# ekzhang/rpt

Hardware: AMD Instinct MI355X
Metric: Msamples/s (higher is better)
Workload: dtype f64

## Files before the change

rpt_amd/csrc/api_render.cpp:

```cpp
#include "api_internal.h"

namespace rptapi {

int event_pair_begin(rptgpu_scene* h, int kind, bool on) {
  h->stats.kernel_launches[kind]++;
  if (!on || h->ev_used + 2 > MAX_EVENT_PAIRS * 2) return -1;
  while ((int)h->ev_pool.size() < h->ev_used + 2) {
    hipEvent_t e;
    HIP_TRY(hipEventCreate(&e));
    h->ev_pool.push_back(e);
  }
  const int e0 = h->ev_used;
  h->ev_used += 2;
  HIP_TRY(hipEventRecord(h->ev_pool[e0], h->stream));
  return e0;
}
void event_pair_end(rptgpu_scene* h, int kind, int e0) {
  if (e0 < 0) return;
  HIP_TRY(hipEventRecord(h->ev_pool[e0 + 1], h->stream));
  h->pending.push_back({kind, e0, e0 + 1});
}

struct Bracket {
  rptgpu_scene* h;
  int kind, e0;
  Bracket(rptgpu_scene* h_, int kind_, bool on) : h(h_), kind(kind_), e0(event_pair_begin(h_, kind_, on)) {}
  void done() { event_pair_end(h, kind, e0); }
};

struct QueryMarks {
  rptgpu_scene* h;
  bool on;
  int e0[RPT_K_COUNT];
  QueryMarks(rptgpu_scene* h_, bool on_) : h(h_), on(on_) {
    for (int& e : e0) e = -1;
  }
};
void query_mark(void* ctx, int kind, int end) {
  QueryMarks* q = (QueryMarks*)ctx;
  if (kind < 0 || kind >= RPT_K_COUNT) return;
  if (!end) {
    q->e0[kind] = event_pair_begin(q->h, kind, q->on);
  } else {
    event_pair_end(q->h, kind, q->e0[kind]);
    q->e0[kind] = -1;
  }
}

void drain_events(rptgpu_scene* h) {
  for (auto& p : h->pending) {
    float ms = 0;
    HIP_TRY(hipEventElapsedTime(&ms, h->ev_pool[p.e0], h->ev_pool[p.e1]));
    h->stats.kernel_ms[p.kind] += ms;
  }
  h->pending.clear();
  h->ev_used = 0;
}

std::vector<uint32_t> pixel_list(uint32_t width, uint32_t height, uint32_t tw, uint32_t th, uint32_t pi, uint32_t pc) {
  std::vector<uint32_t> pix;
  uint32_t tiles_x = (width + tw - 1) / tw;
  pix.reserve((size_t)width * height / pc + 1);
  for (uint32_t by = 0; by < height; by += 8)
    for (uint32_t bx = 0; bx < width; bx += 8)
      for (uint32_t y = by; y < std::min(by + 8, height); y++)
        for (uint32_t x = bx; x < std::min(bx + 8, width); x++) {
          uint32_t tile = (y / th) * tiles_x + (x / tw);
          if (pc <= 1 || tile % pc == pi) pix.push_back(y * width + x);
        }
  return pix;
}
void ensure_partition(rptgpu_scene* h, const RptRenderParams& p) {
  uint32_t tw = p.tile_width ? p.tile_width : 32, th = p.tile_height ? p.tile_height : 8;
  uint32_t pc = p.part_count ? p.part_count : 1, pi = p.part_count ? p.part_index : 0;
  uint32_t key[6] = {p.width, p.height, tw, th, pi, pc};
  if (std::memcmp(key, h->part_key, sizeof key) == 0 && h->pixels.p) return;
  std::vector<uint32_t> pix = pixel_list(p.width, p.height, tw, th, pi, pc);
  h->pixels.upload(pix, h->stream);
  HIP_TRY(hipStreamSynchronize(h->stream));
  h->npix = (uint32_t)pix.size();
  std::memcpy(h->part_key, key, sizeof key);
}

void ensure_generic(rptgpu_scene* h, bool all) {
  const uint32_t blocks_few = 64, blocks_all = (uint32_t)std::max(64, std::min(1024, h->num_cus * 4));
  const uint32_t want = (all ? blocks_all : blocks_few) * 256u;
  if (h->gen_threads < want) {
    const uint64_t levels = std::max(1u, h->gen_levels), frames = std::max(1u, h->gen_frames);
    h->gen_defer.release(); h->gen_frame.release();
    h->gen_defer.alloc(levels * 8u * want);
    h->gen_frame.alloc(frames * 12u * want);
    h->gen_overflow.alloc(1);
    HIP_TRY(hipMemsetAsync(h->gen_overflow.p, 0, sizeof(uint32_t), h->stream));
    h->gen_threads = want;
  }
  h->spill.gen = GenericStack{h->gen_defer.p, h->gen_frame.p, h->gen_threads, std::max(1u, h->gen_levels), std::max(1u, h->gen_frames)};
  h->spill.gen_overflow = h->gen_overflow.p;
  h->spill.gen_blocks_few = blocks_few;
  h->spill.gen_blocks_all = h->gen_threads / 256u >= blocks_all ? blocks_all : blocks_few;
}

int drain_call(rptgpu_scene* h, bool read_overflow) {
  hipStream_t st = h->stream;
  uint32_t gen_overflow = 0;
  if (read_overflow) HIP_TRY(hipMemcpyAsync(&gen_overflow, h->gen_overflow.p, sizeof gen_overflow, hipMemcpyDeviceToHost, st));
  HIP_TRY(hipStreamSynchronize(st));
  drain_events(h);
  if (gen_overflow) {
    (void)hipMemsetAsync(h->gen_overflow.p, 0, sizeof(uint32_t), st);
    return fail(h, RPTGPU_E_TREE_TOO_DEEP, "rpt_tree_generic: the traversal outgrew the stack sized for this scene (internal error)");
  }
  return RPTGPU_OK;
}

void ensure_sort_bufs(rptgpu_scene* h, uint64_t cap) {
  h->sort_kin.alloc(cap); h->sort_kout.alloc(cap); h->sort_vin.alloc(cap);
  size_t bytes = rpt_strict::TABLE.sort_temp_bytes((uint32_t)cap);
  h->sort_tmp.alloc(bytes);
  h->sort_bufs = SortBufs{h->sort_kin.p, h->sort_kout.p, h->sort_vin.p, h->sort_tmp.p, bytes};
}

uint32_t zeros_common(const std::vector<rptdev::Light>& lights) {
  for (const rptdev::Light& l : lights)
    if (l.kind == RPT_LIGHT_DIRECTIONAL && (l.vec[0] == 0.0 || l.vec[1] == 0.0 || l.vec[2] == 0.0)) return 1;
  return 0;
}

void ensure_workspace(rptgpu_scene* h, uint64_t cap, uint64_t rec_cols) {
  if (cap <= h->ws_cap && rec_cols <= h->ws_rec_cols && h->ray.p) return;
  cap = std::max(cap, h->ws_cap);
  rec_cols = std::max(rec_cols, h->ws_rec_cols);
  int nl = std::max(1, h->dscene.num_lights);
  h->ray.alloc(6 * cap);
  h->hit.alloc(4 * cap);
  h->hit_obj.alloc(cap);
  h->draw.alloc(cap); h->pid.alloc(cap); h->col.alloc(cap);
  if (h->path_reorder) {
    h->next_rows.alloc(8 * cap);
  } else {
    h->ray_next.alloc(6 * cap);
    h->draw_next.alloc(cap); h->pid_next.alloc(cap); h->col_next.alloc(cap);
  }
  h->last_col.alloc(cap);
  h->rec.release();
  h->rec.alloc((uint64_t)rptdev::REC_FIELDS * rec_cols);
  h->rec_parent.alloc(rec_cols);
  h->shadow.release();
  h->shadow.alloc((uint64_t)nl * rptdev::SHADOW_FIELDS * cap);
  h->counters.alloc(2 * (2 + (size_t)nl));
  h->shadow_q.release();
  h->shadow_q.alloc((uint64_t)nl * cap);
  h->srt.release();
  h->srt.alloc((uint64_t)nl * cap);
  if (h->has_deep) {
    h->tq.alloc(3 * cap);
    h->tq_ctr.alloc(16);
    {
      const uint64_t threads = (uint64_t)std::max(1, h->num_cus * 4) / 4 * RPT_TT_WAVES * 256;
      const uint64_t levels = (uint64_t)(std::max<uint32_t>((uint32_t)rptdev::KD_MAX_STACK, h->max_tree_depth + 1u) - RPT_TT_LEVELS_MIN);
      h->spill_node.alloc(levels * threads); h->spill_ts.alloc(levels * threads); h->spill_bmax.alloc(levels * threads);
      h->tree_rays.alloc(8 * cap);
      h->spill = StackSpill{h->spill_node.p, h->spill_ts.p, h->spill_bmax.p, (uint32_t)threads, zeros_common(h->host_lights),
                            h->tree_rays.p};
    }
    ensure_generic(h, h->gen_all);
    if (h->sort_rays) ensure_sort_bufs(h, cap);
  }
  if (h->path_reorder) {
    h->path_order.alloc(cap);
    ensure_sort_bufs(h, cap);
  }
  h->ws_cap = cap;
  h->ws_rec_cols = rec_cols;
}

void print_prof(const KernelTable* kt, const char* what) {
  static const char* const NAMES[29] = {
      "tree_trace refill", "tree_trace node steps", "tree_trace box tests", "tree_trace pop", "tree_trace write-out",
      "tree_trace exact tests", "in-kernel node step", "in-kernel box batch", "in-kernel child test",
      "in-kernel triangle batch", "in-kernel object", "paths fetch", "paths raygen", "paths closest_hit",
      "paths illuminate", "paths visible", "paths nee_bsdf", "paths sample_f", "paths bsdf", "paths record",
      "paths fold+store", "flat candidate walk", "fold iteration", "rejection round", "paths fused query",
      "paths draws", "paths shade block", "pre-trace pass", "pre-trace pass, cubes skipped"};
  unsigned long long t[4][29];
  if (!kt->read_prof(t)) return;
  unsigned long long tot = 0;
  for (int i = 0; i < 29; i++) tot += t[0][i];
  std::fprintf(stderr, "prof[%s] %-28s %8s %10s %14s %10s\n", what, "phase", "time %", "lanes/64", "iterations", "lanes/64");
  for (int i = 0; i < 29; i++) {
    if (!t[0][i] && !t[2][i]) continue;
    char a[32] = "-", b[32] = "-", c[32] = "-", d[32] = "-";
    if (t[0][i]) {
      std::snprintf(a, sizeof a, "%.2f", tot ? 100.0 * (double)t[0][i] / (double)tot : 0.0);
      std::snprintf(b, sizeof b, "%.1f", (double)t[1][i] / (double)t[0][i]);
    }
    if (t[2][i]) {
      std::snprintf(c, sizeof c, "%llu", t[2][i]);
      std::snprintf(d, sizeof d, "%.1f", (double)t[3][i] / (double)t[2][i]);
    }
    std::fprintf(stderr, "prof[%s] %-28s %8s %10s %14s %10s\n", what, NAMES[i], a, b, c, d);
  }
}

void release_workspace(rptgpu_scene* h) {
  h->ray.release(); h->ray_next.release(); h->hit.release(); h->hit_obj.release(); h->draw.release(); h->draw_next.release();
  h->pid.release(); h->pid_next.release(); h->col.release(); h->col_next.release(); h->rec.release();
  h->rec_parent.release(); h->last_col.release();
  h->shadow.release(); h->tq.release(); h->srt.release(); h->shadow_q.release();
  h->sort_kin.release(); h->sort_kout.release(); h->sort_vin.release(); h->sort_tmp.release(); h->tree_rays.release();
  h->path_order.release(); h->next_rows.release();
  h->gen_defer.release(); h->gen_frame.release(); h->gen_threads = 0;
  h->ws_cap = 0; h->ws_rec_cols = 0;
}

rptplan::PassPlan size_pass(rptgpu_scene* h, const rptplan::PassInput& in, uint32_t npix, bool generic_all) {
  rptplan::PassPlan pp = rptplan::plan_pass(in);
  for (;;) {
    const uint64_t np = rptplan::pass_slots(npix, pp);
    try {
      ensure_workspace(h, np, rptplan::pass_rec_cols(np, in.ratio));
      if (generic_all) ensure_generic(h, true);
      return pp;
    } catch (const HipError& e) {
      if (e.e != hipErrorOutOfMemory || pp.s_chunk == 1) throw;
      (void)hipGetLastError();
      release_workspace(h);
      h->ws_fail_paths = rptplan::fail_paths_after_oom(h->ws_fail_paths, np);
      pp = rptplan::shrink_after_oom(pp);
    }
  }
}

void reset_tree_counters(rptgpu_scene* h) {
  HIP_TRY(hipMemsetAsync(h->tq_ctr.p, 0, 16 * sizeof(uint32_t), h->stream));
  h->qtune.ctr_set = 0;
}
static void tree_query(rptgpu_scene* h, const KernelTable* kt, const rptdev::PathState& ps, const uint32_t* queue, uint32_t n,
                       int light, double* srt, const uint32_t* d_n, const QueryHook* hook) {
  kt->query(h->stream, h->dscene, ps, queue, n, light, srt, d_n, h->obj_deep.data(), h->obj_tris.data(), h->dscene.num_objects,
            h->tq.p, h->tq_ctr.p, (uint32_t)std::max(1, h->num_cus * 4), h->sort_rays ? &h->sort_bufs : nullptr, hook, &h->spill,
            &h->qtune);
}
void query_closest(rptgpu_scene* h, const KernelTable* kt, const rptdev::PathState& ps, uint32_t n, const QueryHook* hook) {
  tree_query(h, kt, ps, nullptr, n, -1, nullptr, nullptr, hook);
}
void query_visibility(rptgpu_scene* h, const KernelTable* kt, const rptdev::PathState& ps, int l, uint32_t n,
                      const uint32_t* d_n, const QueryHook* hook) {
  tree_query(h, kt, ps, h->shadow_q.p + (uint64_t)l * ps.cap, n, l, h->srt.p, d_n, hook);
}

rptdev::Camera make_camera(const RptCamera& c) {
  rptdev::Camera d{};
  std::memcpy(d.eye, c.eye, sizeof d.eye);
  std::memcpy(d.direction, c.direction, sizeof d.direction);
  std::memcpy(d.up, c.up, sizeof d.up);
  d.d = 1.0 / std::tan(c.fov / 2.0);
  const double* a = c.direction;
  const double* b = c.up;
  double cr[3] = {a[1] * b[2] - a[2] * b[1], a[2] * b[0] - a[0] * b[2], a[0] * b[1] - a[1] * b[0]};
  double len = std::sqrt((cr[0] * cr[0] + cr[1] * cr[1]) + cr[2] * cr[2]);
  for (int k = 0; k < 3; k++) d.right[k] = cr[k] / len;
  d.aperture = c.aperture;
  d.focal_distance = c.focal_distance;
  return d;
}

const char* bad_params(const RptRenderParams* p) {
  if (!p->width || !p->height || !p->iterations) return "width, height and iterations must be non-zero";
  if (p->max_bounces > 254) return "max_bounces > 254";
  if ((uint64_t)p->width * p->height >= (1ull << 31)) return "frame too large";
  if (p->part_count && p->part_index >= p->part_count) return "part_index >= part_count";
  if (p->precision_mode != RPT_PRECISION_F64_STRICT) return BAD_MODE;
  return nullptr;
}

int64_t free_memory() {
  size_t free_b = 0, total_b = 0;
  return hipMemGetInfo(&free_b, &total_b) == hipSuccess ? (int64_t)free_b : -1;
}

rptdev::PathState path_state(rptgpu_scene* h) {
  rptdev::PathState ps{};
  ps.ray = h->ray.p; ps.hit = h->hit.p; ps.hit_obj = h->hit_obj.p; ps.draw = h->draw.p;
  ps.pid = h->pid.p; ps.col = h->col.p;
  ps.ray_next = h->ray_next.p; ps.draw_next = h->draw_next.p; ps.pid_next = h->pid_next.p; ps.col_next = h->col_next.p;
  ps.rec = h->rec.p; ps.rec_parent = h->rec_parent.p; ps.last_col = h->last_col.p;
  ps.shadow = h->shadow.p; ps.cap = h->ws_cap; ps.rec_cap = h->ws_rec_cols;
  if (h->path_reorder) {
    ps.sort_keys = h->sort_kin.p; ps.sort_vals = h->sort_vin.p; ps.next_rows = h->next_rows.p;
    std::memcpy(ps.key_bounds, h->scene_bounds, sizeof ps.key_bounds);
  }
  return ps;
}

void render_persistent(rptgpu_scene* h, const KernelTable* kt, const RptRenderParams& p, rptdev::Frame fr,
                       const rptdev::Camera& cam, void* out, bool out_f32, bool packed, bool prof) {
  hipStream_t st = h->stream;
  const uint32_t npix = fr.npix;
  const bool print_launch = std::getenv("RPTGPU_PRINT_LAUNCH") != nullptr;
  const uint64_t lbuf_held = h->lbuf.n * sizeof(double);
  const int64_t free_b = lbuf_held < h->lbuf_max_bytes ? free_memory() : -1;
  const bool flat = h->all_flat && !h->dscene.force_general;
  FlatLayout lay = flat ? h->flat_layout : FlatLayout{};
  const uint32_t flat_lds = lay.off_end;
  if (RPT_PRETRACE_CULL && lay.pretrace_cull) {
    for (size_t i = 0; i < h->obj_geom.size() && i < 64 && lay.cull_n < (uint32_t)RPT_CULL_MAX; i++) {
      uint32_t r[4];
      if (((lay.cull_always >> i) & 1ull) ||
          !rpthost::pinhole_screen_rect(rpthost::world_box(h->obj_geom[i], h->top_insts[i]), cam, fr.width, fr.height, r))
        continue;
      lay.cull_obj[lay.cull_n] = (uint32_t)i;
      const bool off = r[0] > r[1] || r[2] > r[3];
      lay.cull_lo[lay.cull_n] = off ? 0xffffffffu : (r[0] | (r[2] << 16));
      lay.cull_ext[lay.cull_n] = off ? 0u : ((r[1] - r[0]) | ((r[3] - r[2]) << 16));
      lay.cull_n++;
    }
  }
  const rptplan::PersistentPlan pl = rptplan::plan_persistent(
      npix, p.iterations, p.max_bounces, h->num_cus, kt->paths_max_blocks_per_cu(flat ? &lay : nullptr, flat_lds, false),
      h->lbuf_max_bytes, lbuf_held, free_b, h->paths_chunk, h->all_flat, h->dscene.force_general, h->flat_layout.obj_filter);
  bool park = flat && h->opt.env_park != 0 && h->dscene.env_kind != RPT_ENV_COLOR;
  if (park && kt->paths_max_blocks_per_cu(&lay, flat_lds, true) < pl.per_cu) park = false;
  h->prec.alloc((uint64_t)rpt_fold_ring_slots(p.max_bounces) * rptdev::REC_FIELDS * ((uint64_t)pl.nblocks * 64));
  h->lbuf.alloc(std::max<uint64_t>(1, (uint64_t)pl.spp_l * 3 * npix));
  if (print_launch)
    std::fprintf(stderr, "rpt_paths<%s>: %d blocks/CU x %d CUs -> %u blocks, %u samples per work item, %u launch(es) of %u spp, "
                 "dynamic LDS %u B per wave (the flat scene's tables)%s%s%s%s\n",
                 flat ? (lay.obj_filter ? "KdFlatF" : lay.n_tris ? "KdFlat" : "KdFlatG") : "KdLds", pl.per_cu, h->num_cus, pl.nblocks,
                 pl.chunk, pl.n_launch, pl.spp_l, flat_lds, park ? " + parked environment lookups" : "",
                 flat && lay.n_tris && lay.fuse_query && !park ? ", shadow and bounce rays in one query" : "",
                 flat && lay.n_tris && lay.fuse_query && !park && lay.scene_consts ? ", a hit's scene constants from the wave's tables" : "",
                 RPT_HIT_POOL && flat && lay.n_tris && lay.fuse_query && !park ? ", pre-traced hits in a wave-level pool" : "");
  h->counters.alloc(4);
  h->pcounters.alloc(16);
  HIP_TRY(hipMemsetAsync(h->pcounters.p, 0, 16 * sizeof(unsigned long long), st));
  for (uint32_t s0 = 0; s0 < p.iterations; s0 += pl.spp_l) {
    const uint32_t spp = std::min(pl.spp_l, p.iterations - s0);
    const uint64_t items = rptplan::work_items(npix, spp, pl.chunk);
    fr.sample_base = p.sample_index_base + s0;
    HIP_TRY(hipMemsetAsync(h->counters.p, 0, sizeof(uint32_t), st));
    { Bracket b(h, RPT_K_PATHS, prof);
      kt->paths(st, h->dscene, fr, cam, h->counters.p, h->prec.p, h->pcounters.p, h->lbuf.p, spp, pl.chunk, (uint32_t)items,
                pl.nblocks, lay, flat, flat_lds, park, h->opt.paths_batch);
      b.done(); }
    kt->sum_samples(st, fr, h->lbuf.p, spp, s0 == 0);
    if (print_launch) {
      uint32_t ended = 0;
      HIP_TRY(hipMemcpyAsync(&ended, h->counters.p, sizeof ended, hipMemcpyDeviceToHost, st));
      HIP_TRY(hipStreamSynchronize(st));
      const uint32_t batch_used = h->opt.paths_batch ? std::min<uint32_t>(h->opt.paths_batch, RPT_PATHS_BATCH_MAX)
                                                      : std::min(256u, std::max((uint32_t)items / (std::max(1u, pl.nblocks) * 32u), 16u));
      std::fprintf(stderr, "rpt_paths work counter: ended at %u for %llu items; %u waves, claims of at most %u: dead claims %lld of at most %llu\n",
                   ended, (unsigned long long)items, pl.nblocks, batch_used, (long long)ended - (long long)items,
                   (unsigned long long)pl.nblocks * (64u + batch_used));
    }
  }
  HIP_TRY(hipGetLastError());
  kt->finish(st, fr, (double)p.iterations, std::pow(2.0, p.exposure_value), out, out_f32, packed);
  unsigned long long rc[16] = {0};
  HIP_TRY(hipMemcpyAsync(rc, h->pcounters.p, sizeof rc, hipMemcpyDeviceToHost, st));
  HIP_TRY(hipStreamSynchronize(st));
  if (std::getenv("RPTGPU_PRINT_PHASES")) print_prof(kt, "rpt_paths");
  h->stats.samples += (uint64_t)npix * p.iterations;
  h->stats.extend_rays += rc[0];
  h->stats.shadow_rays += rc[1];
  h->stats.shadow_rays_traced += rc[1];
}

bool run_pass(rptgpu_scene* h, const KernelTable* kt, const RptRenderParams& p, const rptdev::Frame& fr,
              const RaySource& src, uint32_t n_paths, uint32_t spp, bool prof, const QueryHook& qhook, uint64_t* cols) {
  hipStream_t st = h->stream;
  rptdev::PathState ps = path_state(h);
  const int nlights = h->dscene.num_lights;
  const uint32_t nctr = 2u + (uint32_t)nlights;
  HIP_TRY(hipMemsetAsync(h->counters.p, 0, 2 * (size_t)nctr * sizeof(uint32_t), st));
  uint32_t cset = 0;
  if (h->has_deep) reset_tree_counters(h);
  { Bracket b(h, RPT_K_RAYGEN, prof);
    if (src.cam) kt->raygen(st, fr, *src.cam, ps, n_paths);
    else if (src.probe >= 0) kt->raygen_probes(st, fr, src.origins, src.dirs, (uint32_t)src.probe, src.ids_out, src.id_base, ps, n_paths);
    else kt->raygen_rays(st, fr, src.origins, src.dirs, src.first_draw, src.ids_out, src.id_base, ps, n_paths);
    b.done(); }
  h->stats.samples += n_paths;
  uint32_t n_active = n_paths;
  const uint32_t* const queue = nullptr;
  uint32_t* const next = nullptr;
  uint64_t rec_off = 0;
  const bool by_object = h->has_deep && (!(p.flags & RPT_FLAG_GENERAL_TRAVERSAL) || h->tree_kids);
  for (uint32_t depth = 0; depth <= p.max_bounces && n_active; depth++) {
    if (rec_off + n_active > h->ws_rec_cols) {
      *cols = rec_off + n_active;
      return false;
    }
    { Bracket b(h, RPT_K_EXTEND, prof);
      if (by_object)
        query_closest(h, kt, ps, n_active, &qhook);
      else
        kt->extend(st, h->dscene, ps, queue, n_active);
      b.done(); }
    h->stats.extend_rays += n_active;
    uint32_t* const ctrs = h->counters.p + (size_t)cset * nctr;
    uint32_t* const ctrs_next = h->counters.p + (size_t)(cset ^ 1u) * nctr;
    cset ^= 1u;
    { Bracket b(h, RPT_K_SHADE, prof);
      kt->shade(st, h->dscene, fr, ps, queue, n_active, depth, next, ctrs, h->shadow_q.p, ctrs_next, nctr, (uint32_t)rec_off); b.done(); }
    h->cnt_host.resize(2 + (size_t)nlights);
    uint32_t* cnt = h->cnt_host.data();
    HIP_TRY(hipMemcpyAsync(cnt, ctrs, (2 + (size_t)nlights) * sizeof(uint32_t), hipMemcpyDeviceToHost, st));
    HIP_TRY(hipStreamSynchronize(st));
    for (int l = 0; l < nlights; l++) h->stats.shadow_rays_traced += cnt[2 + l];
    if (prof && h->pending.size() >= 256) drain_events(h);
    h->stats.shadow_rays += (uint64_t)cnt[1] * (uint64_t)h->dscene.num_shadow_lights;
    if (nlights > 0) {
      Bracket b(h, RPT_K_SHADOW, prof);
      if (by_object) {
        for (int l = 0; l < nlights; l++)
          if (h->light_casts[l] && cnt[2 + l]) query_visibility(h, kt, ps, l, cnt[2 + l], ctrs + 2 + l, &qhook);
      } else {
        uint32_t n_max = 0;
        for (int l = 0; l < nlights; l++)
          if (h->light_casts[l]) n_max = std::max(n_max, cnt[2 + l]);
        if (n_max) kt->shadow_rays(st, h->dscene, ps, h->shadow_q.p, ctrs + 2, n_max, nlights, h->srt.p);
      }
      kt->shadow_sum(st, h->dscene, ps, queue, n_active, (uint32_t)rec_off, h->srt.p);
      b.done();
    }
    rec_off += n_active;
    n_active = cnt[0];
    if (h->path_reorder) {
      if (n_active && depth < p.max_bounces) {
        Bracket b(h, RPT_K_TREE_SORT, prof);
        kt->path_reorder(st, ps, n_active, n_active >= h->path_reorder_min, &h->sort_bufs, h->path_order.p);
        b.done();
      }
    } else {
      std::swap(ps.ray, ps.ray_next); std::swap(ps.draw, ps.draw_next); std::swap(ps.pid, ps.pid_next); std::swap(ps.col, ps.col_next);
    }
  }
  { Bracket b(h, RPT_K_RESOLVE, prof);
    if (src.probe >= 0) kt->resolve_probes(st, fr, ps, spp, (uint32_t)src.probe);
    else kt->resolve(st, fr, ps, spp);
    b.done(); }
  HIP_TRY(hipGetLastError());
  *cols = rec_off;
  return true;
}

rptplan::PassInput pass_input(rptgpu_scene* h, uint32_t npix, uint32_t iterations) {
  rptplan::PassInput in{};
  in.npix = npix; in.iterations = iterations;
  in.per_slot = rptplan::wavefront_slot_bytes(h->dscene.num_lights, h->has_deep, h->sort_rays, h->path_reorder);
  in.target_paths = h->target_paths; in.budget_bytes = h->ws_budget_bytes;
  in.free_percent = RPT_WS_FREE_PERCENT;
  if (const char* e = std::getenv("RPTGPU_WS_FREE_FRACTION")) in.free_percent = (uint64_t)std::min(95, std::max(5, std::atoi(e)));
  return in;
}
void pass_input_now(rptgpu_scene* h, rptplan::PassInput& in) {
  in.free_bytes = in.target_paths ? -1 : free_memory();
  in.held_slots = h->ws_cap; in.held_cols = h->ws_rec_cols;
  in.fail_paths = h->ws_fail_paths;
}

void render_wavefront(rptgpu_scene* h, const KernelTable* kt, const RptRenderParams& p, rptdev::Frame fr,
                      const RaySource& src, void* out, bool out_f32, bool packed, bool prof) {
  hipStream_t st = h->stream;
  const uint32_t npix = fr.npix;
  const bool print_launch = std::getenv("RPTGPU_PRINT_LAUNCH") != nullptr;
  if (h->rec_ratio_bounces != p.max_bounces) {
    h->rec_ratio = 0.0; h->rec_ratio_bounces = p.max_bounces;
    if (const char* e = std::getenv("RPTGPU_REC_RATIO")) h->rec_ratio = std::max(0.0, std::atof(e));
  }
  rptplan::PassInput in = pass_input(h, npix, p.iterations);
  const bool generic_all = h->has_deep && (h->gen_all || h->dscene.force_general);
  const uint32_t acc_w = src.probe >= 0 ? probe_width((uint32_t)src.probe) : 3u;
  HIP_TRY(hipMemsetAsync(h->accum.p, 0, (uint64_t)npix * acc_w * sizeof(double), st));
  QueryMarks qm(h, prof);
  const QueryHook qhook{query_mark, &qm};

  for (uint32_t s0 = 0; s0 < p.iterations;) {
    in.remaining = p.iterations - s0;
    in.rec_ratio = h->rec_ratio;
    in.ratio = rptplan::pass_ratio(h->rec_ratio, p.max_bounces);
    pass_input_now(h, in);
    const rptplan::PassPlan pp = size_pass(h, in, npix, generic_all);
    const uint32_t n_paths = npix * pp.s_chunk;
    fr.sample_base = p.sample_index_base + s0;
    const RptStats stats_at_start = h->stats;
    uint64_t cols = 0;
    if (!run_pass(h, kt, p, fr, src, n_paths, pp.s_chunk, prof, qhook, &cols)) {
      HIP_TRY(hipStreamSynchronize(st));
      h->stats = stats_at_start;
      h->rec_ratio = rptplan::ratio_after_restart(h->rec_ratio, cols, n_paths, p.max_bounces);
      if (print_launch)
        std::fprintf(stderr, "wavefront pass of %u spp started over: the record pool (%.2f columns per path) ran out; now %.2f\n", pp.s_chunk, in.ratio, h->rec_ratio);
      continue;
    }
    h->rec_ratio = rptplan::ratio_after_pass(h->rec_ratio, cols, n_paths);
    if (print_launch)
      std::fprintf(stderr, "wavefront pass: %u spp, %u paths, %llu record columns used of %llu (%.3f per path, pool sized for %.3f)\n",
                   pp.s_chunk, n_paths, (unsigned long long)cols, (unsigned long long)h->ws_rec_cols, (double)cols / (double)n_paths, in.ratio);
    s0 += pp.s_chunk;
  }
  if (src.probe >= 0) kt->finish_probes(st, fr, acc_w, src.probe_scale, (double*)out);
  else kt->finish(st, fr, (double)p.iterations, std::pow(2.0, p.exposure_value), out, out_f32, packed);
  if (std::getenv("RPTGPU_PRINT_PHASES")) {
    HIP_TRY(hipStreamSynchronize(st));
    print_prof(kt, "wavefront");
  }
}

int render_impl(rptgpu_scene* h, const RptCamera* camera, const RptRenderParams* p, void* d_out, bool out_f32,
                double* host_out, hipStream_t user_stream, bool packed, const uint32_t* d_list, uint32_t n_list) {
  if (!h || !camera || !p) return fail(h, RPTGPU_E_INVALID_ARGUMENT, "null argument");
  REFUSE_IF_ABANDONED(h);
  if (const char* why = bad_params(p)) return fail(h, RPTGPU_E_INVALID_ARGUMENT, why);
  if (d_list && (!packed || !d_out || host_out)) return fail(h, RPTGPU_E_INVALID_ARGUMENT, "a pixel list renders packed into device memory");
  auto t0 = std::chrono::steady_clock::now();
  const int rc = guarded(h, h->device, [&]() -> int {
    struct EventPairs {
      rptgpu_scene* h;
      ~EventPairs() { h->pending.clear(); h->ev_used = 0; }
    } event_pairs{h};
    (void)hipGetLastError();
    hipStream_t st = h->stream;
    const KernelTable* kt = table_for(p->precision_mode, h->ext_shapes);
    const bool prof = (p->flags & RPT_FLAG_PROFILE_KERNELS) != 0;
    if (!d_list) ensure_partition(h, *p);
    const uint32_t npix = d_list ? n_list : h->npix;
    const uint64_t frame_elems = (uint64_t)p->width * p->height * 3;
    const size_t out_elem = out_f32 ? sizeof(float) : sizeof(double);
    void* out = d_out;
    if (!out) {
      h->out_full.alloc(frame_elems);
      out = h->out_full.p;
    }
    if (user_stream) HIP_TRY(hipStreamSynchronize(user_stream));
    if (!packed) HIP_TRY(hipMemsetAsync(out, 0, frame_elems * out_elem, st));
    const bool wavefront = use_wavefront(h, p->flags, h->prefer_wavefront);
    h->dscene.force_general = (p->flags & RPT_FLAG_GENERAL_TRAVERSAL) ? 1 : 0;
    if (npix) {
      h->accum.alloc((uint64_t)npix * 3);
      rptdev::Frame fr{};
      fr.width = p->width; fr.height = p->height; fr.npix = npix; fr.pixels = d_list ? d_list : h->pixels.p;
      fr.max_bounces = p->max_bounces; fr.seed = p->seed; fr.accum = h->accum.p;
      const rptdev::Camera cam = make_camera(*camera);
      RaySource src{};
      src.cam = &cam;
      if (wavefront) render_wavefront(h, kt, *p, fr, src, out, out_f32, packed, prof);
      else render_persistent(h, kt, *p, fr, cam, out, out_f32, packed, prof);
    }
    HIP_TRY(hipGetLastError());
    if (host_out) HIP_TRY(hipMemcpyAsync(host_out, out, frame_elems * out_elem, hipMemcpyDeviceToHost, st));
    return drain_call(h, wavefront && h->has_deep && h->gen_overflow.p);
  });
  if (rc != RPTGPU_OK) return rc;
  h->stats.total_ms += std::chrono::duration<double, std::milli>(std::chrono::steady_clock::now() - t0).count();
  return RPTGPU_OK;
}

}

extern "C" {

int rptgpu_render_batch(rptgpu_scene* h, const RptCamera* camera, const RptRenderParams* params, double* out_rgb) {
  if (!out_rgb) return fail(h, RPTGPU_E_INVALID_ARGUMENT, "null out_rgb");
  return render_impl(h, camera, params, nullptr, false, out_rgb, nullptr);
}

int rptgpu_render_batch_device(rptgpu_scene* h, const RptCamera* camera, const RptRenderParams* params, void* d_out,
                               int out_is_f32, void* stream) {
  if (!d_out) return fail(h, RPTGPU_E_INVALID_ARGUMENT, "null d_out");
  return render_impl(h, camera, params, d_out, out_is_f32 != 0, nullptr, (hipStream_t)stream);
}

int rptgpu_closest_hit(rptgpu_scene* h, uint64_t n, const double* origins, const double* dirs,
                       uint32_t precision_mode, double* out_t, double* out_normal, int32_t* out_object) {
  if (!h || (n && (!origins || !dirs || !out_t || !out_normal || !out_object)))
    return fail(h, RPTGPU_E_INVALID_ARGUMENT, "null argument");
  if (precision_mode != RPT_PRECISION_F64_STRICT) return fail(h, RPTGPU_E_INVALID_ARGUMENT, BAD_MODE);
  REFUSE_IF_ABANDONED(h);
  if (!n) return RPTGPU_OK;
  return guarded(h, h->device, [&]() -> int {
    hipStream_t st = h->stream;
    if (h->has_deep && (!h->rays_in_kernel || h->tree_kids)) {
      const KernelTable* kt = table_for(precision_mode, h->ext_shapes);
      const uint64_t piece = std::min<uint64_t>(n, 4ull << 20);
      ensure_workspace(h, piece, piece);
      const rptdev::PathState ps = path_state(h);
      std::vector<double> soa(6 * piece), hit(4 * piece);
      for (uint64_t base = 0; base < n; base += piece) {
        const uint64_t m = std::min(piece, n - base);
        for (uint64_t i = 0; i < m; i++)
          for (int k = 0; k < 3; k++) {
            soa[(uint64_t)k * m + i] = origins[3 * (base + i) + k];
            soa[(uint64_t)(3 + k) * m + i] = dirs[3 * (base + i) + k];
          }
        for (int k = 0; k < 6; k++)
          HIP_TRY(hipMemcpyAsync(ps.ray + (uint64_t)k * ps.cap, soa.data() + (uint64_t)k * m, m * sizeof(double), hipMemcpyHostToDevice, st));
        reset_tree_counters(h);
        query_closest(h, kt, ps, (uint32_t)m, nullptr);
        HIP_TRY(hipGetLastError());
        for (int k = 0; k < 4; k++)
          HIP_TRY(hipMemcpyAsync(hit.data() + (uint64_t)k * m, ps.hit + (uint64_t)k * ps.cap, m * sizeof(double), hipMemcpyDeviceToHost, st));
        HIP_TRY(hipMemcpyAsync(out_object + base, ps.hit_obj, m * sizeof(int32_t), hipMemcpyDeviceToHost, st));
        HIP_TRY(hipStreamSynchronize(st));
        for (uint64_t i = 0; i < m; i++) {
          out_t[base + i] = hit[i];
          for (int k = 0; k < 3; k++) out_normal[3 * (base + i) + k] = hit[(uint64_t)(1 + k) * m + i];
        }
      }
      return drain_call(h, h->gen_overflow.p != nullptr);
    }
    DevBuf<double> d_o, d_d, d_t, d_n;
    DevBuf<int32_t> d_obj;
    d_o.alloc(3 * n); d_d.alloc(3 * n); d_t.alloc(n); d_n.alloc(3 * n); d_obj.alloc(n);
    HIP_TRY(hipMemcpyAsync(d_o.p, origins, 3 * n * sizeof(double), hipMemcpyHostToDevice, st));
    HIP_TRY(hipMemcpyAsync(d_d.p, dirs, 3 * n * sizeof(double), hipMemcpyHostToDevice, st));
    table_for(precision_mode, h->ext_shapes)->extend_rays(st, h->dscene, d_o.p, d_d.p, n, d_t.p, d_n.p, d_obj.p);
    HIP_TRY(hipGetLastError());
    HIP_TRY(hipMemcpyAsync(out_t, d_t.p, n * sizeof(double), hipMemcpyDeviceToHost, st));
    HIP_TRY(hipMemcpyAsync(out_normal, d_n.p, 3 * n * sizeof(double), hipMemcpyDeviceToHost, st));
    HIP_TRY(hipMemcpyAsync(out_object, d_obj.p, n * sizeof(int32_t), hipMemcpyDeviceToHost, st));
    HIP_TRY(hipStreamSynchronize(st));
    return RPTGPU_OK;
  });
}

int rptgpu_eval_math(rptgpu_scene* h, int fn, uint64_t n, const double* x, const double* y, double* out) {
  if (!h || (n && (!x || !out)) || fn < 0 || fn > 7 || (fn >= 6 && n && !y))
    return fail(h, RPTGPU_E_INVALID_ARGUMENT, "bad argument");
  if (!n) return RPTGPU_OK;
  return guarded(h, h->device, [&]() -> int {
    DevBuf<double> dx, dy, dout;
    dx.alloc(n); dy.alloc(n); dout.alloc(n);
    HIP_TRY(hipMemcpyAsync(dx.p, x, n * sizeof(double), hipMemcpyHostToDevice, h->stream));
    if (y) HIP_TRY(hipMemcpyAsync(dy.p, y, n * sizeof(double), hipMemcpyHostToDevice, h->stream));
    else HIP_TRY(hipMemsetAsync(dy.p, 0, n * sizeof(double), h->stream));
    rpt_strict::TABLE.eval_math(h->stream, fn, n, dx.p, dy.p, dout.p);
    HIP_TRY(hipGetLastError());
    HIP_TRY(hipMemcpyAsync(out, dout.p, n * sizeof(double), hipMemcpyDeviceToHost, h->stream));
    HIP_TRY(hipStreamSynchronize(h->stream));
    return RPTGPU_OK;
  });
}

}
```

rpt_amd/csrc/kernels.h:

```cpp
#pragma once
#include <hip/hip_runtime.h>
#include <stdint.h>

#include "device_types.h"
#include "hit_pool.h"
#include "launch_limits.h"

#ifndef RPT_FLAT_RUN
#define RPT_FLAT_RUN 6
#endif

#define RPT_PATHS_WAVE_LDS 20480u
#define RPT_PATHS_WALKER_LDS 2560u
#ifndef RPT_RAY_STASH
#define RPT_RAY_STASH 2
#endif
#ifndef RPT_FUSE_QUERY
#define RPT_FUSE_QUERY 1
#endif
#ifndef RPT_SHADE_SPLIT
#define RPT_SHADE_SPLIT 1
#endif
#ifndef RPT_PRETRACE_CULL
#define RPT_PRETRACE_CULL 1
#endif
#define RPT_CULL_MAX 4
#ifndef RPT_SCENE_CONSTS
#define RPT_SCENE_CONSTS 7
#endif
#define RPT_MAT_CONSTS_BYTES 88u
#define RPT_CUBE_NORMALS_BYTES 144u
#define RPT_PATHS_STASH_LDS 4864u
#define RPT_PATHS_STASH_HIT_LDS 6656u
#ifndef RPT_HIT_POOL
#define RPT_HIT_POOL 1
#endif
#ifndef RPT_POOL_CAP
#define RPT_POOL_CAP 64u
#endif
#ifndef RPT_POOL_REFILL
#define RPT_POOL_REFILL 56u
#endif
#define RPT_PATHS_POOL_LDS (RPT_POOL_CAP * 100u)
static_assert(RPT_POOL_CAP >= 64u && RPT_POOL_REFILL >= 1u && RPT_POOL_REFILL <= RPT_POOL_CAP,
              "a refill of 64 lanes has to fit an empty pool, and a full pool has to fall to the refill mark");
static_assert(RPT_PATHS_POOL_LDS <= RPT_PATHS_STASH_HIT_LDS, "the host's fit checks leave room for RayStashHit only");
#define RPT_PATHS_STASH_MAX_LDS (RPT_RAY_STASH >= 2 ? RPT_PATHS_STASH_HIT_LDS : RPT_PATHS_STASH_LDS)
#ifndef RPT_PARK_K
#define RPT_PARK_K 4
#endif
#define RPT_PATHS_PARK_LDS (RPT_PARK_K * 2624u)
#ifndef RPT_PATH_REORDER_MIN
#define RPT_PATH_REORDER_MIN (1u << 20)
#endif

#define RPT_RETIRE_ITEMS 16u
#define RPT_RETIRE_TILE (RPT_RETIRE_ITEMS * 256u)

struct FlatLayout {
  uint32_t off_tris, off_refs, off_mat, off_leaf;
  uint32_t off_end;
  uint32_t n_refs, n_tris;
  uint32_t off_qtab, plane_cnt;
  const double* plane_vals;
  uint32_t obj_filter;
  uint32_t off_obox;
  const rptdev::LeafBox* obj_box;
  const double* obj_grid;
  uint64_t obj_always;
  uint32_t fuse_query;
  uint32_t pretrace_cull, cull_n;
  uint64_t cull_always;
  uint32_t cull_obj[RPT_CULL_MAX], cull_lo[RPT_CULL_MAX], cull_ext[RPT_CULL_MAX];
  uint32_t scene_consts, off_consts;
};

struct SortBufs {
  uint32_t *keys_in, *keys_out, *vals_in;
  void* tmp;
  size_t tmp_bytes;
};

#ifndef RPT_TT_WAVES
#define RPT_TT_WAVES 4
#endif
#ifndef RPT_TT_LEVELS
#define RPT_TT_LEVELS 7
#endif
#define RPT_TT_LEVELS_MIN RPT_TT_LEVELS
struct GenericStack {
  double* defer;
  double* frame;
  uint32_t threads, levels, frames;
};
struct StackSpill {
  uint32_t* node;
  double* ts;
  double* bmax;
  uint32_t threads;
  uint32_t zeros_common;
  double* rays;
  GenericStack gen;
  uint32_t* gen_overflow;
  uint32_t gen_blocks_few, gen_blocks_all;
};

struct QueryHook {
  void (*mark)(void* ctx, int kind, int end);
  void* ctx;
};

struct QueryTuning {
  uint32_t ctr_set;
  uint32_t sort_min_rays;
};

struct KernelTable {
  void (*raygen)(hipStream_t, const rptdev::Frame&, const rptdev::Camera&, const rptdev::PathState&, uint32_t n_paths);
  void (*raygen_rays)(hipStream_t, const rptdev::Frame&, const double* origins, const double* dirs, uint32_t first_draw,
                      uint32_t* ids_out, uint32_t id_base, const rptdev::PathState&, uint32_t n_paths);
  void (*extend)(hipStream_t, const rptdev::Scene&, const rptdev::PathState&, const uint32_t* queue, uint32_t n);
  void (*extend_rays)(hipStream_t, const rptdev::Scene&, const double* o, const double* d, uint64_t n, double* out_t,
                      double* out_n, int32_t* out_obj);
  void (*shade)(hipStream_t, const rptdev::Scene&, const rptdev::Frame&, const rptdev::PathState&,
                const uint32_t* queue, uint32_t n, uint32_t depth, uint32_t* next_queue, uint32_t* counters, uint32_t* sq,
                uint32_t* zero_next , uint32_t zero_n,
                uint32_t rec_off );
  void (*shadow_rays)(hipStream_t, const rptdev::Scene&, const rptdev::PathState&, const uint32_t* sq_all,
                      const uint32_t* sq_counts, uint32_t n_max, int num_lights, double* srt);
  void (*resolve)(hipStream_t, const rptdev::Frame&, const rptdev::PathState&, uint32_t n_samples);
  void (*finish)(hipStream_t, const rptdev::Frame&, double iterations, double ev_scale, void* out, bool f32, bool packed);
  void (*scatter_f32)(hipStream_t, const float* src, const uint32_t* pixels, uint32_t n, float* dst);
  void (*eval_math)(hipStream_t, int fn, uint64_t n, const double* x, const double* y, double* out);
  int (*paths_max_blocks_per_cu)(const FlatLayout* flat , uint32_t lds_bytes, bool park);
  void (*paths)(hipStream_t, const rptdev::Scene&, const rptdev::Frame&, const rptdev::Camera&,
                uint32_t* work_counter, double* rec, unsigned long long* ray_counters, double* lbuf, uint32_t spp,
                uint32_t chunk, uint32_t n_items, uint32_t nblocks, const FlatLayout& lay, bool flat, uint32_t lds_bytes,
                bool park, uint32_t batch );
  void (*sum_samples)(hipStream_t, const rptdev::Frame&, const double* lbuf, uint32_t spp, bool first);
  void (*query)(hipStream_t, const rptdev::Scene&, const rptdev::PathState&, const uint32_t* queue, uint32_t n,
                int light, double* srt, const uint32_t* n_dev , const uint8_t* obj_deep, const uint8_t* obj_tris, int num_objects,
                uint32_t* tq, uint32_t* tq_ctr, uint32_t trace_blocks, const SortBufs* sort, const QueryHook* hook,
                const StackSpill* spill , QueryTuning* qt);
  size_t (*sort_temp_bytes)(uint32_t n);
  void (*shadow_sum)(hipStream_t, const rptdev::Scene&, const rptdev::PathState&, const uint32_t* queue, uint32_t n,
                     uint32_t rec_off, const double* srt);
  void (*buffer_accumulate)(hipStream_t, double* total, double* frame, const double* packed, const uint32_t* list,
                            uint32_t n, uint32_t* counts, double* mean, double* m2);
  void (*buffer_retire)(hipStream_t, const uint32_t* list, uint32_t n, const uint32_t* counts, const double* mean,
                        const double* m2, uint32_t min_batches, double abs_tol, double rel_tol, uint8_t* keep,
                        uint32_t* block_cnt, uint32_t* out_list, uint32_t* out_n);
  void (*buffer_image)(hipStream_t, const double* total, const uint32_t* counts, uint32_t w, uint32_t h, uint32_t radius,
                       const double* thr, uint8_t* out);
  void (*buffer_variance)(hipStream_t, const double* total, const double* const* batches, const uint32_t* counts,
                          uint64_t npix, double* out);
  bool (*read_prof)(unsigned long long out[4][29]);
  void (*path_reorder)(hipStream_t, const rptdev::PathState&, uint32_t n, bool sorted, const SortBufs* sort, uint32_t* order);
  void (*aov)(hipStream_t, const rptdev::Scene&, const rptdev::Frame&, const rptdev::Camera&, const rptdev::AovOut&,
              uint32_t iterations);
  void (*aov_fold)(hipStream_t, const rptdev::Scene&, const rptdev::Frame&, const rptdev::PathState&, const rptdev::AovOut&,
                   uint32_t spp, bool first);
  void (*denoise_prepare)(hipStream_t, const double* total, const uint32_t* counts, const double* m2, const rptdev::AovOut& feat,
                          uint32_t w, uint32_t h, uint64_t stride, double* c_out, double* v_out, double* g_normal,
                          double* g_position, double* g_albedo, double* g_depth, uint8_t* g_hit);
  void (*denoise_level)(hipStream_t, const rptdev::DenoiseGuide&, const double* c_in, const double* v_in, double* c_out,
                        double* v_out, uint32_t step, const rptdev::DenoiseSigmas&);
  void (*denoise_finish)(hipStream_t, const double* c_in, uint64_t stride, uint64_t npix, const double* thr, double* out_linear,
                         uint8_t* out_rgb8);
  void (*raygen_probes)(hipStream_t, const rptdev::Frame&, const double* positions, const double* normals, uint32_t kind,
                        uint32_t* ids_out, uint32_t id_base, const rptdev::PathState&, uint32_t n_paths);
  void (*resolve_probes)(hipStream_t, const rptdev::Frame&, const rptdev::PathState&, uint32_t n_samples, uint32_t kind);
  void (*finish_probes)(hipStream_t, const rptdev::Frame&, uint32_t width, double scale, double* out);
};

namespace rpt_strict { extern const KernelTable TABLE; }
namespace rpt_strict_ext { extern const KernelTable TABLE; }
```

rpt_amd/csrc/kernels/buffer.inc:

```

__global__ void __launch_bounds__(256) rpt_buffer_accumulate(double* __restrict__ total, double* __restrict__ frame,
                                                             const double* __restrict__ packed,
                                                             const uint32_t* __restrict__ list, uint32_t n,
                                                             uint32_t* __restrict__ counts, double* __restrict__ mean,
                                                             double* __restrict__ m2) {
  const uint32_t i = blockIdx.x * blockDim.x + threadIdx.x;
  if (i >= n) return;
  const uint64_t p = list ? (uint64_t)list[i] : (uint64_t)i;
  D3 x;
  if (list) {
    x = ld3(packed + 3 * (uint64_t)i);
    frame[3 * p] = x.x; frame[3 * p + 1] = x.y; frame[3 * p + 2] = x.z;
  } else {
    x = ld3(frame + 3 * p);
  }
  const D3 t = ld3(total + 3 * p) + x;
  total[3 * p] = t.x; total[3 * p + 1] = t.y; total[3 * p + 2] = t.z;
  const uint32_t c = counts[p] + 1u;
  counts[p] = c;
  const D3 m0 = ld3(mean + 3 * p);
  const D3 d = x - m0;
  const D3 m = m0 + d / (double)c;
  mean[3 * p] = m.x; mean[3 * p + 1] = m.y; mean[3 * p + 2] = m.z;
  m2[p] = m2[p] + dot(d, x - m);
}

RPT_DEV bool stays_active(uint32_t p, const uint32_t* __restrict__ counts, const double* __restrict__ mean,
                          const double* __restrict__ m2, uint32_t min_batches, double abs_tol, double rel_tol) {
  const uint32_t n = counts[p];
  const D3 m = ld3(mean + 3 * (uint64_t)p);
  const double e = (m2[p] / ((double)n - 1.0)) / (double)n;
  const double t = abs_tol + rel_tol * ((m.x + m.y) + m.z);
  return !(n >= min_batches && e <= t * t);
}
__global__ void __launch_bounds__(256) rpt_retire_count(const uint32_t* __restrict__ list, uint32_t n,
                                                        const uint32_t* __restrict__ counts, const double* __restrict__ mean,
                                                        const double* __restrict__ m2, uint32_t min_batches, double abs_tol,
                                                        double rel_tol, uint8_t* __restrict__ keep,
                                                        uint32_t* __restrict__ block_cnt) {
  __shared__ uint32_t s_cnt[4];
  const uint32_t lane = threadIdx.x & 63u, wave = threadIdx.x >> 6;
  const uint32_t tile = blockIdx.x * RPT_RETIRE_TILE;
  uint32_t cnt = 0;
  for (uint32_t k = 0; k < RPT_RETIRE_ITEMS; k++) {
    const uint32_t i = tile + k * 256u + threadIdx.x;
    bool kp = false;
    if (i < n) {
      kp = stays_active(list[i], counts, mean, m2, min_batches, abs_tol, rel_tol);
      keep[i] = kp ? 1 : 0;
    }
    cnt += (uint32_t)__popcll(__ballot(kp));
  }
  if (lane == 0) s_cnt[wave] = cnt;
  __syncthreads();
  if (threadIdx.x == 0) block_cnt[blockIdx.x] = (s_cnt[0] + s_cnt[1]) + (s_cnt[2] + s_cnt[3]);
}
__global__ void __launch_bounds__(256) rpt_retire_scatter(const uint32_t* __restrict__ list, uint32_t n,
                                                          const uint8_t* __restrict__ keep,
                                                          const uint32_t* __restrict__ block_cnt,
                                                          uint32_t* __restrict__ out_list, uint32_t* __restrict__ out_n) {
  __shared__ uint32_t s_sum[256];
  __shared__ uint32_t s_cnt[4];
  const uint32_t lane = threadIdx.x & 63u, wave = threadIdx.x >> 6;
  uint32_t sum = 0;
  for (uint32_t j = threadIdx.x; j < blockIdx.x; j += 256u) sum += block_cnt[j];
  s_sum[threadIdx.x] = sum;
  __syncthreads();
  for (uint32_t s = 128u; s > 0; s >>= 1) {
    if (threadIdx.x < s) s_sum[threadIdx.x] += s_sum[threadIdx.x + s];
    __syncthreads();
  }
  uint32_t off = s_sum[0];
  const uint32_t tile = blockIdx.x * RPT_RETIRE_TILE;
  const uint64_t below = (1ull << lane) - 1ull;
  for (uint32_t k = 0; k < RPT_RETIRE_ITEMS; k++) {
    const uint32_t i = tile + k * 256u + threadIdx.x;
    const bool kp = i < n && keep[i] != 0;
    const uint64_t mask = __ballot(kp);
    if (lane == 0) s_cnt[wave] = (uint32_t)__popcll(mask);
    __syncthreads();
    uint32_t wave_off = 0;
    for (uint32_t w = 0; w < wave; w++) wave_off += s_cnt[w];
    if (kp) out_list[off + wave_off + (uint32_t)__popcll(mask & below)] = list[i];
    off += (s_cnt[0] + s_cnt[1]) + (s_cnt[2] + s_cnt[3]);
    __syncthreads();
  }
  if (blockIdx.x == gridDim.x - 1 && threadIdx.x == 0) *out_n = off;
}

__global__ void __launch_bounds__(256) rpt_buffer_image(const double* __restrict__ total,
                                                        const uint32_t* __restrict__ counts, uint32_t w, uint32_t h,
                                                        uint32_t radius, const double* __restrict__ thr,
                                                        uint8_t* __restrict__ out) {
  uint32_t p = blockIdx.x * blockDim.x + threadIdx.x;
  if (p >= w * h) return;
  uint32_t y = p / w, x = p - y * w;
  D3 color = mk(0, 0, 0);
  uint64_t count = 0;
  uint32_t i0 = x >= radius ? x - radius : 0, j0 = y >= radius ? y - radius : 0;
  for (uint32_t i = i0; i <= x + radius; i++)
    for (uint32_t j = j0; j <= y + radius; j++)
      if (i < w && j < h) {
        color = color + ld3(total + 3 * ((uint64_t)j * w + i));
        count += counts[(uint64_t)j * w + i];
      }
  D3 c = color / (double)count;
  double v[3] = {c.x, c.y, c.z};
  for (int ch = 0; ch < 3; ch++) {
    double t = fmin(fmax(v[ch], 0.0), 1.0);
    int lo = 0, hi = 255;
    while (lo < hi) {
      int mid = (lo + hi + 1) >> 1;
      if (thr[mid] <= t) lo = mid;
      else hi = mid - 1;
    }
    out[3 * (uint64_t)p + ch] = (uint8_t)lo;
  }
}

__global__ void __launch_bounds__(256) rpt_buffer_variance(const double* __restrict__ total,
                                                           const double* const* __restrict__ batches,
                                                           const uint32_t* __restrict__ counts, uint64_t npix,
                                                           double* __restrict__ out) {
  uint64_t p = (uint64_t)blockIdx.x * blockDim.x + threadIdx.x;
  if (p >= npix) return;
  const uint32_t nb = counts[p];
  D3 mean = ld3(total + 3 * p) / (double)nb;
  double ss = 0.0;
  for (uint32_t b = 0; b < nb; b++) {
    D3 dlt = ld3(batches[b] + 3 * p) - mean;
    ss += dot(dlt, dlt);
  }
  out[p] = ss / ((double)nb - 1.0);
}

__global__ void __launch_bounds__(256) rpt_eval_math(int fn, uint64_t n, const double* __restrict__ x,
                                                     const double* __restrict__ y, double* __restrict__ out) {
  uint64_t i = (uint64_t)blockIdx.x * blockDim.x + threadIdx.x;
  if (i >= n) return;
  double s, c;
  switch (fn) {
    case 0: out[i] = rptc_exp(x[i]); break;
    case 1: out[i] = rpt_log(x[i]); break;
    case 2: out[i] = rptc_atan(x[i]); break;
    case 3: rptc_sincos_pio2(x[i], &s, &c); out[i] = s; break;
    case 4: rptc_sincos_pio2(x[i], &s, &c); out[i] = c; break;
    case 5: out[i] = rptc_acos(x[i]); break;
    case 6: out[i] = rptc_atan2(y[i], x[i]); break;
    default: {
      RcpD rc = rcp_make(x[i]);
      double a = fabs(y[i]);
      out[i] = (rc.ok && safe_range(a, a)) ? div_fast(y[i], rc) : y[i] / x[i];
      break;
    }
  }
}

template __global__ void rpt_paths<KdLds, false>(Scene, Frame, Camera, PersistArgs);
template __global__ void rpt_paths<KdFlat, false>(Scene, Frame, Camera, PersistArgs);
template __global__ void rpt_paths<KdFlat, true>(Scene, Frame, Camera, PersistArgs);
#if RPT_FUSE_QUERY && RPT_RAY_STASH >= 2
template __global__ void rpt_paths<KdFlat, false, true>(Scene, Frame, Camera, PersistArgs);
#if RPT_SCENE_CONSTS
template __global__ void rpt_paths<KdFlat, false, true, true>(Scene, Frame, Camera, PersistArgs);
#endif
#endif
template __global__ void rpt_paths<KdFlatG, false>(Scene, Frame, Camera, PersistArgs);
template __global__ void rpt_paths<KdFlatG, true>(Scene, Frame, Camera, PersistArgs);
template __global__ void rpt_paths<KdFlatF, false>(Scene, Frame, Camera, PersistArgs);
template __global__ void rpt_paths<KdFlatF, true>(Scene, Frame, Camera, PersistArgs);
template __global__ void rpt_rays_objects<false, KdLdsW>(Scene, RayBatch, const uint32_t*, uint32_t, int, int);
template __global__ void rpt_rays_objects<true, KdLdsW>(Scene, RayBatch, const uint32_t*, uint32_t, int, int);
template __global__ void rpt_rays_objects<false, KdFlat>(Scene, RayBatch, const uint32_t*, uint32_t, int, int);
template __global__ void rpt_rays_objects<true, KdFlat>(Scene, RayBatch, const uint32_t*, uint32_t, int, int);
#ifdef RPT_EXT_SHAPES
template __global__ void rpt_nest_trace<false>(Scene, RayBatch, int, const uint32_t*, const uint32_t*, const uint32_t*, uint32_t*, uint32_t*, StackSpill);
template __global__ void rpt_nest_trace<true>(Scene, RayBatch, int, const uint32_t*, const uint32_t*, const uint32_t*, uint32_t*, uint32_t*, StackSpill);
#endif
template __global__ void rpt_tree_enter<false>(Scene, RayBatch, const uint32_t*, uint32_t, int, uint32_t*, uint32_t*, uint32_t*, uint32_t*, uint32_t*, uint32_t*, uint32_t*, double*, uint32_t);
template __global__ void rpt_tree_enter<true>(Scene, RayBatch, const uint32_t*, uint32_t, int, uint32_t*, uint32_t*, uint32_t*, uint32_t*, uint32_t*, uint32_t*, uint32_t*, double*, uint32_t);
template __global__ void rpt_tree_trace<true, false, false>(Scene, RayBatch, int, const uint32_t*, const uint32_t*, const uint32_t*, uint32_t*, uint32_t*, uint32_t*, StackSpill);
template __global__ void rpt_tree_trace<true, false, true>(Scene, RayBatch, int, const uint32_t*, const uint32_t*, const uint32_t*, uint32_t*, uint32_t*, uint32_t*, StackSpill);
template __global__ void rpt_tree_trace<true, true, false>(Scene, RayBatch, int, const uint32_t*, const uint32_t*, const uint32_t*, uint32_t*, uint32_t*, uint32_t*, StackSpill);
template __global__ void rpt_tree_trace<true, true, true>(Scene, RayBatch, int, const uint32_t*, const uint32_t*, const uint32_t*, uint32_t*, uint32_t*, uint32_t*, StackSpill);
template __global__ void rpt_tree_trace<false, false, false>(Scene, RayBatch, int, const uint32_t*, const uint32_t*, const uint32_t*, uint32_t*, uint32_t*, uint32_t*, StackSpill);
template __global__ void rpt_tree_trace<false, false, true>(Scene, RayBatch, int, const uint32_t*, const uint32_t*, const uint32_t*, uint32_t*, uint32_t*, uint32_t*, StackSpill);
template __global__ void rpt_tree_trace<false, true, false>(Scene, RayBatch, int, const uint32_t*, const uint32_t*, const uint32_t*, uint32_t*, uint32_t*, uint32_t*, StackSpill);
template __global__ void rpt_tree_trace<false, true, true>(Scene, RayBatch, int, const uint32_t*, const uint32_t*, const uint32_t*, uint32_t*, uint32_t*, uint32_t*, StackSpill);
template __global__ void rpt_tree_generic<false>(Scene, RayBatch, int, const uint32_t*, const uint32_t*, GenericStack, uint32_t*, uint32_t*);
template __global__ void rpt_tree_generic<true>(Scene, RayBatch, int, const uint32_t*, const uint32_t*, GenericStack, uint32_t*, uint32_t*);
template __global__ void rpt_finish<float>(Frame, double, double, float*, int);
template __global__ void rpt_finish<double>(Frame, double, double, double*, int);
```

rpt_amd/csrc/kernels/paths.inc:

```

#ifndef RPT_PARK_FLUSH
#define RPT_PARK_FLUSH 160
#endif
struct ParkLds {
  double d[RPT_PARK_K][3][64];
  uint32_t u[RPT_PARK_K][4][64];
  uint8_t list[RPT_PARK_K * 64];
};
static_assert(sizeof(ParkLds) == RPT_PATHS_PARK_LDS, "kernels.h sizes the wave's LDS budget with it");
static_assert(RPT_PARK_K >= 1 && RPT_PARK_K <= 4, "two bits for the entry in ParkLds::list, three for a lane's count");
struct PersistArgs {
  uint32_t* work_counter;
  double* rec;
  unsigned long long* ray_counters;
  double* lbuf;
  uint32_t spp;
  uint32_t chunk;
  uint32_t n_items;
  uint32_t nthreads;
  uint32_t ring;
  uint32_t batch;
  uint32_t park_off;
  FlatLayout flat;
};

#ifndef RPT_PATHS_WAVES
#define RPT_PATHS_WAVES 2
#endif
template <class LDS> struct PathsLds { using type = LDS; };
template <> struct PathsLds<KdFlat> { struct type { int unused; }; };
struct KdFlatG { static constexpr int levels = 0; };
template <> struct PathsLds<KdFlatG> { struct type { int unused; }; };
struct KdFlatF { static constexpr int levels = 0; };
template <> struct PathsLds<KdFlatF> { struct type { int unused; }; };
RPT_DEV void camera_ray(const Frame& fr, const Camera& cam, double dim, uint32_t pix, uint32_t smp, D3& ro, D3& rd, Rng& rr) {
  uint32_t y = pix / fr.width, x = pix - y * fr.width;
  double xn = ((double)(2 * x + 1) - (double)fr.width) / dim;
  double yn = ((double)(2 * (fr.height - y) - 1) - (double)fr.height) / dim;
  rr = rng_make(fr.seed, pix, fr.sample_base + smp, 0);
  double dx = gen_range(rr, -1.0 / dim, 1.0 / dim);
  double dy = gen_range(rr, -1.0 / dim, 1.0 / dim);
  double px = xn + dx, py = yn + dy;
  D3 direction = ld3(cam.direction), up = ld3(cam.up), right = ld3(cam.right);
  ro = ld3(cam.eye);
  D3 new_dir = cam.d * direction + px * right + py * up;
  if (cam.aperture > 0.0) {
    D3 focal_point = ro + normalize(new_dir) * cam.focal_distance;
    double a, b;
    unit_disc(rr, a, b);
    ro = ro + (a * right + b * up) * cam.aperture;
    new_dir = focal_point - ro;
  }
  rd = normalize(new_dir);
}
struct ItemPool { uint32_t next, end, seen; };
RPT_DEV bool fetch_item(const PersistArgs& pa, const Frame& fr, uint32_t lane, bool want, ItemPool& pool, uint32_t& f_p_local,
                        uint32_t& f_pixel, uint32_t& f_s, uint32_t& f_s_end) {
  bool got = false;
  const uint64_t need_mask = __ballot(want);
  if (need_mask) {
    const uint32_t n = (uint32_t)__popcll(need_mask), rank = (uint32_t)__popcll(need_mask & ((1ull << lane) - 1ull));
    const uint32_t avail = pool.end - pool.next;
    uint32_t idx = pool.next + rank;
    if (n > avail) {
      const uint32_t left = pa.n_items - min(pa.n_items, pool.seen);
      const uint32_t more = max(n - avail, min(pa.batch, left / (pa.nthreads >> 4)));
      uint32_t base = 0;
      if (lane == (uint32_t)__ffsll((long long)need_mask) - 1u) base = atomicAdd(pa.work_counter, more);
      base = (uint32_t)__builtin_amdgcn_readfirstlane((int)__shfl(base, __ffsll((long long)need_mask) - 1));
      if (rank >= avail) idx = base + (rank - avail);
      pool.next = base + (n - avail);
      pool.end = base + more;
      pool.seen = pool.end;
    } else {
      pool.next += n;
    }
    if (want && idx < pa.n_items) {
      uint32_t c = idx / fr.npix;
      f_p_local = idx - c * fr.npix;
      f_pixel = fr.pixels[f_p_local];
      f_s = c * pa.chunk;
      f_s_end = min(f_s + pa.chunk, pa.spp);
      got = true;
    }
  }
  return got;
}
RPT_DEV uint32_t next_header_slot(uint32_t b, uint32_t depth, uint32_t ring) {
  uint32_t nb = b + depth + 1u;
  if (nb >= ring) nb -= ring;
  return nb;
}
RPT_DEV uint32_t rec_slot(uint32_t fold_st, uint32_t depth, uint32_t ring) {
  return next_header_slot(fold_st >> 16, depth, ring);
}
RPT_DEV void rec_store_bsdf(double* r, const D3& f, double inv_pdf, double abscos) {
  r[3] = f.x; r[4] = f.y; r[5] = f.z; r[6] = inv_pdf; r[7] = abscos;
}
RPT_DEV void path_ended(const PersistArgs& pa, const Frame& fr, double* __restrict__ rec, double (*fold_l)[64],
                        uint32_t (*fold_u)[64], uint32_t lane, uint32_t& fold_st, const D3& A, uint32_t depth, uint32_t b,
                        uint32_t s, uint32_t p_local) {
  if (depth == 0) {
    double* lb = pa.lbuf + (uint64_t)s * 3 * fr.npix + p_local;
    lb[0] = A.x;
    lb[fr.npix] = A.y;
    lb[2 * (uint64_t)fr.npix] = A.z;
  } else if ((fold_st & 0xffffu) == 0u) {
    fold_l[0][lane] = A.x; fold_l[1][lane] = A.y; fold_l[2][lane] = A.z;
    fold_u[0][lane] = depth; fold_u[1][lane] = b; fold_u[2][lane] = s; fold_u[3][lane] = p_local;
    fold_st |= depth;
  } else {
    double* r = rec + b * REC_FIELDS;
    r[0] = A.x; r[1] = A.y; r[2] = A.z;
    r[3] = __longlong_as_double((long long)((uint64_t)s | ((uint64_t)p_local << 32)));
    r[4] = __longlong_as_double((long long)depth);
  }
}
RPT_DEV void park_push(ParkLds& park, uint32_t lane, uint32_t& pcnt, uint32_t& park_hd, uint32_t& park_recs, uint32_t& fold_st,
                       uint32_t ring, const D3& d, uint32_t depth, uint32_t s, uint32_t p_local) {
  const uint32_t k = pcnt, b = fold_st >> 16;
  park.d[k][0][lane] = d.x; park.d[k][1][lane] = d.y; park.d[k][2][lane] = d.z;
  park.u[k][0][lane] = depth; park.u[k][1][lane] = b; park.u[k][2][lane] = s; park.u[k][3][lane] = p_local;
  if (depth != 0u) {
    if (park_hd == 0xffffffffu) park_hd = b;
    park_recs += depth;
    fold_st = (fold_st & 0xffffu) | (next_header_slot(b, depth, ring) << 16);
  }
  pcnt = k + 1u;
}
struct RayStash {
  double v[7][64];
  uint32_t u[5][64];
};
static_assert(sizeof(RayStash) == RPT_PATHS_STASH_LDS, "kernels.h sizes the wave's LDS budget with it");
struct RayStashHit {
  double v[10][64];
  uint32_t u[6][64];
};
static_assert(sizeof(RayStashHit) == RPT_PATHS_STASH_HIT_LDS, "kernels.h sizes the wave's LDS budget with it");
template <class S> RPT_DEV void stash_put_pos(S& st, uint32_t lane, const D3& o) {
  st.v[0][lane] = o.x; st.v[1][lane] = o.y; st.v[2][lane] = o.z;
}
template <class S> RPT_DEV void stash_put_dir(S& st, uint32_t lane, const D3& d) {
  st.v[3][lane] = d.x; st.v[4][lane] = d.y; st.v[5][lane] = d.z;
}
template <class S> RPT_DEV void stash_put_ray(S& st, uint32_t lane, const D3& o, const D3& d) {
  stash_put_pos(st, lane, o);
  stash_put_dir(st, lane, d);
}
template <class S> RPT_DEV void stash_take_ray(const S& st, uint32_t lane, D3& o, D3& d) {
  o = mk(st.v[0][lane], st.v[1][lane], st.v[2][lane]);
  d = mk(st.v[3][lane], st.v[4][lane], st.v[5][lane]);
}
template <class S> RPT_DEV void stash_swap_ray(S& st, uint32_t lane, D3& o, D3& d) {
  D3 so, sd;
  stash_take_ray(st, lane, so, sd);
  stash_put_ray(st, lane, o, d);
  o = so; d = sd;
}
template <class S> RPT_DEV void stash_put_path(S& st, uint32_t lane, uint32_t p_local, uint32_t pixel, uint32_t s, uint32_t s_end, const Rng& r) {
  st.v[6][lane] = __longlong_as_double((long long)r.hi);
  st.u[0][lane] = p_local; st.u[1][lane] = pixel; st.u[2][lane] = s; st.u[3][lane] = s_end;
  st.u[4][lane] = r.draw;
}
template <class S> RPT_DEV void stash_take_path(const S& st, uint32_t lane, const Frame& fr, uint32_t& p_local, uint32_t& pixel, uint32_t& s,
                             uint32_t& s_end, Rng& r) {
  p_local = st.u[0][lane]; pixel = st.u[1][lane]; s = st.u[2][lane]; s_end = st.u[3][lane];
  r = rng_make(fr.seed, pixel, fr.sample_base + s, 0);
  r.draw = st.u[4][lane];
  r.hi = (uint64_t)__double_as_longlong(st.v[6][lane]);
}
RPT_DEV void stash_put_hit(RayStashHit& st, uint32_t lane, const D3& pos, const D3& nrm, int obj) {
  stash_put_pos(st, lane, pos);
  st.v[7][lane] = nrm.x; st.v[8][lane] = nrm.y; st.v[9][lane] = nrm.z;
  st.u[5][lane] = (uint32_t)obj;
}
RPT_DEV void stash_take_hit(const RayStashHit& st, uint32_t lane, D3& pos, D3& d, D3& nrm, int& obj) {
  stash_take_ray(st, lane, pos, d);
  nrm = mk(st.v[7][lane], st.v[8][lane], st.v[9][lane]);
  obj = (int)st.u[5][lane];
}
struct HitPool {
  double v[10][RPT_POOL_CAP];
  uint32_t u[5][RPT_POOL_CAP];
};
static_assert(sizeof(HitPool) == RPT_PATHS_POOL_LDS, "kernels.h sizes the wave's LDS budget with it");
RPT_DEV void pool_put(HitPool& hp, uint32_t slot, const D3& pos, const D3& d, const D3& nrm, int obj, uint32_t p_local,
                      uint32_t pixel, uint32_t s, const Rng& r) {
  hp.v[0][slot] = pos.x; hp.v[1][slot] = pos.y; hp.v[2][slot] = pos.z;
  hp.v[3][slot] = d.x; hp.v[4][slot] = d.y; hp.v[5][slot] = d.z;
  hp.v[6][slot] = __longlong_as_double((long long)r.hi);
  hp.v[7][slot] = nrm.x; hp.v[8][slot] = nrm.y; hp.v[9][slot] = nrm.z;
  hp.u[0][slot] = (uint32_t)obj; hp.u[1][slot] = p_local; hp.u[2][slot] = pixel; hp.u[3][slot] = s; hp.u[4][slot] = r.draw;
}
RPT_DEV void pool_take(const HitPool& hp, uint32_t slot, const Frame& fr, D3& pos, D3& d, D3& nrm, int& obj, uint32_t& p_local,
                       uint32_t& s, Rng& r) {
  pos = mk(hp.v[0][slot], hp.v[1][slot], hp.v[2][slot]);
  d = mk(hp.v[3][slot], hp.v[4][slot], hp.v[5][slot]);
  nrm = mk(hp.v[7][slot], hp.v[8][slot], hp.v[9][slot]);
  obj = (int)hp.u[0][slot]; p_local = hp.u[1][slot]; s = hp.u[3][slot];
  r = rng_make(fr.seed, hp.u[2][slot], fr.sample_base + s, 0);
  r.draw = hp.u[4][slot];
  r.hi = (uint64_t)__double_as_longlong(hp.v[6][slot]);
}
#ifndef RPT_STASH_REFILL_MIN
#define RPT_STASH_REFILL_MIN 32
#endif
RPT_DEV void end_path(const PersistArgs& pa, const Frame& fr, double* __restrict__ rec, double (*fold_l)[64],
                      uint32_t (*fold_u)[64], uint32_t lane, uint32_t& fold_st, uint32_t ring, const D3& A, uint32_t depth,
                      uint32_t s, uint32_t p_local) {
  const uint32_t b = fold_st >> 16;
  path_ended(pa, fr, rec, fold_l, fold_u, lane, fold_st, A, depth, b, s, p_local);
  if (depth != 0u) fold_st = (fold_st & 0xffffu) | (next_header_slot(b, depth, ring) << 16);
}
template <bool PARK>
RPT_DEV void walker_step(const PersistArgs& pa, const Frame& fr, const double* __restrict__ rec, double (*fold_l)[64],
                         uint32_t (*fold_u)[64], uint32_t lane, uint32_t& fold_st, uint32_t ring, uint32_t park_hd,
                         double probe_chk ) {
  const uint32_t wk = fold_st & 0xffffu, cb = fold_st >> 16;
  const uint32_t wD = fold_u[0][lane], wb = fold_u[1][lane];
  uint32_t pos = wb + wk;
  if (pos >= ring) pos -= ring;
  const uint32_t nh = next_header_slot(wb, wD, ring);
  const bool last = wk == 1u, more = last && nh != cb && (!PARK || nh != park_hd);
  double v[REC_FIELDS], hd[5] = {0.0, 0.0, 0.0, 0.0, 0.0};
#ifdef RPT_PROBE_NO_RING
  (void)pos;
#pragma unroll
  for (int q = 0; q < REC_FIELDS; q++) v[q] = probe_chk * (double)(q + 1);
#else
  {
    const double* r = rec + pos * REC_FIELDS;
#pragma unroll
    for (int q = 0; q < REC_FIELDS; q++) v[q] = r[q];
  }
#endif
  if (more) {
    const double* r = rec + nh * REC_FIELDS;
#pragma unroll
    for (int q = 0; q < 5; q++) hd[q] = r[q];
  }
  D3 L = mk(fold_l[0][lane], fold_l[1][lane], fold_l[2][lane]);
  D3 Ak = mk(v[0], v[1], v[2]);
  D3 f = mk(v[3], v[4], v[5]);
  D3 indirect = v[6] * cmul(f, L) * v[7];
  L = mk(Ak.x + fmin(indirect.x, FIREFLY_CLAMP), Ak.y + fmin(indirect.y, FIREFLY_CLAMP),
         Ak.z + fmin(indirect.z, FIREFLY_CLAMP));
  if (!last) {
    fold_l[0][lane] = L.x; fold_l[1][lane] = L.y; fold_l[2][lane] = L.z;
    fold_st -= 1u;
  } else {
    double* lb = pa.lbuf + (uint64_t)fold_u[2][lane] * 3 * fr.npix + fold_u[3][lane];
    lb[0] = L.x;
    lb[fr.npix] = L.y;
    lb[2 * (uint64_t)fr.npix] = L.z;
    uint32_t nk = 0u;
    if (more) {
      const uint64_t sp = (uint64_t)__double_as_longlong(hd[3]);
      nk = (uint32_t)__double_as_longlong(hd[4]);
      fold_l[0][lane] = hd[0]; fold_l[1][lane] = hd[1]; fold_l[2][lane] = hd[2];
      fold_u[0][lane] = nk; fold_u[1][lane] = nh; fold_u[2][lane] = (uint32_t)sp; fold_u[3][lane] = (uint32_t)(sp >> 32);
    }
    fold_st = (cb << 16) | nk;
  }
}
template <class LDS, bool PARK ,
          bool FUSE = false ,
          bool CONSTS = false >
__global__ void __launch_bounds__(64, RPT_PATHS_WAVES) rpt_paths(Scene sc, Frame fr, Camera cam, PersistArgs pa) {
  extern __shared__ __attribute__((aligned(16))) unsigned char flat_smem[];
  __shared__ typename PathsLds<LDS>::type kd_store;
  LDS* kd_ldsp = reinterpret_cast<LDS*>(&kd_store);
  constexpr bool FILTERED = std::is_same<LDS, KdFlatF>::value;
  constexpr bool IS_FLAT = std::is_same<LDS, KdFlat>::value || std::is_same<LDS, KdFlatG>::value || FILTERED;
  constexpr bool TRIS_IN_LDS = std::is_same<LDS, KdFlat>::value;
  FlatLds fl{};
  if constexpr (IS_FLAT) {
    const FlatLayout& lay = pa.flat;
    const uint32_t l = threadIdx.x;
    TriX* l_lrec = reinterpret_cast<TriX*>(flat_smem);
    Tri* l_tris = reinterpret_cast<Tri*>(flat_smem + lay.off_tris);
    uint32_t* l_refs = reinterpret_cast<uint32_t*>(flat_smem + lay.off_refs);
    Material* l_mat = reinterpret_cast<Material*>(flat_smem + lay.off_mat);
    uint32_t(*l_leaf)[4] = reinterpret_cast<uint32_t(*)[4]>(flat_smem + lay.off_leaf);
    const double* src = reinterpret_cast<const double*>(sc.lrec);
    double* dst = reinterpret_cast<double*>(l_lrec);
    for (uint32_t i = l; i < lay.n_refs * (uint32_t)(sizeof(TriX) / 8); i += 64) dst[i] = src[i];
    if constexpr (TRIS_IN_LDS) {
      src = reinterpret_cast<const double*>(sc.tris);
      dst = reinterpret_cast<double*>(l_tris);
      for (uint32_t i = l; i < lay.n_tris * (uint32_t)(sizeof(Tri) / 8); i += 64) dst[i] = src[i];
    }
    for (uint32_t i = l; i < lay.n_refs; i += 64) l_refs[i] = sc.refs[i];
    for (uint32_t i = l; i < (uint32_t)sc.num_objects * (uint32_t)(sizeof(Material) / 8); i += 64) {
      uint32_t ob = i / (uint32_t)(sizeof(Material) / 8), w = i - ob * (uint32_t)(sizeof(Material) / 8);
      reinterpret_cast<double*>(l_mat)[i] = reinterpret_cast<const double*>(sc.materials + sc.insts[ob].material)[w];
    }
    for (uint32_t ob = l; ob < (uint32_t)sc.num_objects; ob += 64) {
      const Inst& in = sc.insts[ob];
      uint32_t e0 = 0, e1 = 0, e2 = 0, e3 = 0;
      if (in.kind == RPT_SHAPE_MESH) {
        const Tree& tr = sc.trees[in.tree];
        e0 = tr.ref_base; e1 = tr.prim_base; e2 = tr.root_first; e3 = tr.root_leaf - 1u;
      }
      l_leaf[ob][0] = e0; l_leaf[ob][1] = e1; l_leaf[ob][2] = e2; l_leaf[ob][3] = e3;
      if constexpr (FILTERED) {
        l_leaf[ob][3] = e3 | ((uint32_t)in.kind << 8) | (in.has_xf ? 1u << 16 : 0u);
        double* ob6 = reinterpret_cast<double*>(flat_smem + lay.off_obox) + 6u * ob;
        for (int k = 0; k < 6; k++) ob6[k] = in.bounds[k];
      }
    }
    if constexpr (CONSTS) {
      static_assert(FUSE, "the tables serve the fused form");
      scene_consts_fill(sc, sc.tris, l, flat_smem + lay.off_consts);
      fl.consts = flat_smem + lay.off_consts;
    }
    __syncthreads();
    sc.lrec = l_lrec;
    if constexpr (TRIS_IN_LDS) sc.tris = l_tris;
    sc.refs = l_refs;
    fl.lrec = l_lrec; fl.tris = sc.tris; fl.refs = l_refs; fl.obj_mat = l_mat; fl.obj_leaf = l_leaf;
    fl.qtab = reinterpret_cast<double*>(flat_smem + lay.off_qtab);
    fl.plane_vals = lay.plane_vals;
    fl.plane_cnt = lay.plane_cnt;
    if constexpr (FILTERED) {
      fl.obox = reinterpret_cast<const double*>(flat_smem + lay.off_obox);
      fl.obj_box = lay.obj_box; fl.obj_grid = lay.obj_grid; fl.obj_always = lay.obj_always;
    }
  }
  const uint32_t tid = blockIdx.x * blockDim.x + threadIdx.x;
  const uint32_t lane = __lane_id();
  double* __restrict__ rec = pa.rec + (uint64_t)tid * pa.ring * REC_FIELDS;
  __shared__ double fold_l[3][64];
  __shared__ uint32_t fold_u[4][64];
  uint32_t fold_st = 0;
  const uint32_t ring = pa.ring;
  uint32_t p_local = 0, pixel = 0, s = 0, s_end = 0, depth = 0;
  bool done = false, in_path = false;
  D3 o = mk(0, 0, 0), d = mk(0, 0, 1);
  Rng rng = rng_make(fr.seed, 0, 0, 0);
  uint32_t n_ext = 0, n_sh = 0;
#ifdef RPT_PROBE_NO_RING
  double probe_chk = 0.0;
#else
  constexpr double probe_chk = 0.0;
#endif
  const double dim = (double)max(fr.width, fr.height);
  constexpr bool STASH = RPT_RAY_STASH && std::is_same<LDS, KdFlat>::value;
  constexpr bool PRETRACE = STASH && RPT_RAY_STASH >= 2 && !PARK;
  static_assert(!FUSE || PRETRACE, "the fused form is a form of the pre-traced kernel");
  constexpr bool POOL = FUSE && RPT_HIT_POOL != 0;
  using StashT = typename std::conditional<POOL, HitPool, typename std::conditional<PRETRACE, RayStashHit, RayStash>::type>::type;
  __shared__ typename std::conditional<STASH, StashT, int>::type stash_store;
  auto& stash = *reinterpret_cast<StashT*>(&stash_store);
  struct PoolState { uint32_t g_p_local = 0, g_s = ~0u; uint32_t head = 0, cnt = 0; };
  struct NoPoolState {};
  [[maybe_unused]] typename std::conditional<POOL, PoolState, NoPoolState>::type ps;
  bool stash_valid = false, exhausted = false;
  bool pend = false;
#if RPT_PRETRACE_CULL
  uint32_t near = ~0u;
#endif
  ItemPool pool{0u, 0u, 0u};
  constexpr bool park_on = PARK;
  ParkLds& park = *reinterpret_cast<ParkLds*>(flat_smem + (park_on ? pa.park_off : 0u));
  uint32_t pcnt = 0, park_hd = 0xffffffffu, park_recs = 0;
  D3 nx_pos = mk(0, 0, 0), nx_nrm = mk(0, 0, 0);
  int nx_obj = -1;
  PROF_INIT();

  for (;;) {
    if constexpr (POOL) {
      const uint32_t n_need = (uint32_t)__popcll(__ballot(!in_path || nx_obj < 0));
      const uint64_t work_mask = __ballot(!exhausted);
      if (work_mask != 0ull && rpt_pool_refill(ps.cnt, n_need, RPT_POOL_CAP, RPT_POOL_REFILL)) {
        const bool turn = !exhausted && rpt_pool_rank(work_mask, lane) < rpt_pool_gen_limit(ps.cnt, RPT_POOL_CAP);
        const bool want_item = turn && ps.g_s == ~0u;
        uint32_t f_pixel = 0, f_s_end = 0;
        const bool got = fetch_item(pa, fr, lane, want_item, pool, ps.g_p_local, f_pixel, ps.g_s, f_s_end);
        if (want_item && !got) exhausted = true;
        PROF_PHASE(PF_P_FETCH);
        const bool gen = turn && !exhausted;
        const uint64_t gen_mask = __ballot(gen);
        if (gen) {
          const uint32_t g_pixel = fr.pixels[ps.g_p_local];
          D3 go, gd;
          Rng gr;
          camera_ray(fr, cam, dim, g_pixel, ps.g_s, go, gd, gr);
          PROF_PHASE(PF_P_RAYGEN);
          double t = INF;
          D3 hn = mk(0, 0, 0);
#if RPT_PRETRACE_CULL
          const uint64_t skip = cull_skip_mask(pa.flat, cull_near(pa.flat, g_pixel, fr.width));
          PROF_COUNT(PF_P_PRETRACE);
          const int ho = flat_query<false, true, CONSTS>(sc, &fl, go, gd, -INF, t, hn, skip);
#else
          const int ho = flat_query<false, false, CONSTS>(sc, &fl, go, gd, -INF, t, hn);
#endif
          n_ext++;
          if (ho < 0) hn = env_color(sc, gd);
          pool_put(stash, rpt_pool_slot(ps.head, ps.cnt + rpt_pool_rank(gen_mask, lane), RPT_POOL_CAP), go + t * gd, gd, hn, ho,
                   ps.g_p_local, g_pixel, ps.g_s, gr);
          ps.g_s++;
          if (ps.g_s % pa.chunk == 0u || ps.g_s == pa.spp) ps.g_s = ~0u;
          PROF_PHASE(PF_P_HIT);
        }
        rpt_pool_after_push(ps.cnt, gen_mask);
        __syncthreads();
      }
      done = !in_path && exhausted;
      if (ps.cnt == 0u && __ballot(!done || (fold_st & 0xffffu) != 0u) == 0) break;
    } else if constexpr (STASH) {
      bool refill = __ballot(!in_path && !stash_valid && !exhausted) != 0ull;
      if constexpr (PRETRACE) refill = refill || __popcll(__ballot(!stash_valid && !exhausted)) >= RPT_STASH_REFILL_MIN;
      if (refill) {
        const bool gen = !stash_valid && !exhausted;
        uint32_t g_p_local = p_local, g_pixel = pixel, g_s = s + (in_path ? 1u : 0u), g_s_end = s_end;
        const bool want_item = gen && g_s >= g_s_end;
        const bool got = fetch_item(pa, fr, lane, want_item, pool, g_p_local, g_pixel, g_s, g_s_end);
        if (want_item && !got) exhausted = true;
        PROF_PHASE(PF_P_FETCH);
        if (gen && !exhausted) {
          D3 go, gd;
          Rng gr;
          camera_ray(fr, cam, dim, g_pixel, g_s, go, gd, gr);
#if RPT_PRETRACE_CULL
          if constexpr (FUSE) near = cull_near(pa.flat, g_pixel, fr.width);
#endif
          stash_put_ray(stash, lane, go, gd);
          stash_put_path(stash, lane, g_p_local, g_pixel, g_s, g_s_end, gr);
          stash_valid = true;
          pend = PRETRACE;
        }
        PROF_PHASE(PF_P_RAYGEN);
      }
      if (!PRETRACE && !in_path && stash_valid) {
        stash_take_ray(stash, lane, o, d);
        stash_take_path(stash, lane, fr, p_local, pixel, s, s_end, rng);
        stash_valid = false;
        depth = 0;
        in_path = true;
      }
      done = !in_path && exhausted && !(PRETRACE && stash_valid);
      if (__ballot(!done || (fold_st & 0xffffu) != 0u || pcnt != 0u) == 0) break;
    } else {
      const bool need = !done && !in_path && s == s_end;
      if (!fetch_item(pa, fr, lane, need, pool, p_local, pixel, s, s_end) && need) done = true;
      if (__ballot(!done || (fold_st & 0xffffu) != 0u || pcnt != 0u) == 0) break;
      PROF_PHASE(PF_P_FETCH);
      if (!done && !in_path) {
        uint32_t y = pixel / fr.width, x = pixel - y * fr.width;
        double xn = ((double)(2 * x + 1) - (double)fr.width) / dim;
        double yn = ((double)(2 * (fr.height - y) - 1) - (double)fr.height) / dim;
        rng = rng_make(fr.seed, pixel, fr.sample_base + s, 0);
        double dx = gen_range(rng, -1.0 / dim, 1.0 / dim);
        double dy = gen_range(rng, -1.0 / dim, 1.0 / dim);
        double px = xn + dx, py = yn + dy;
        D3 direction = ld3(cam.direction), up = ld3(cam.up), right = ld3(cam.right);
        o = ld3(cam.eye);
        D3 new_dir = cam.d * direction + px * right + py * up;
        if (cam.aperture > 0.0) {
          D3 focal_point = o + normalize(new_dir) * cam.focal_distance;
          double a, b;
          unit_disc(rng, a, b);
          o = o + (a * right + b * up) * cam.aperture;
          new_dir = focal_point - o;
        }
        d = normalize(new_dir);
        depth = 0;
        in_path = true;
      }
    }

    PROF_PHASE(PF_P_RAYGEN);
    bool ending = false, esc = false;
    D3 A_end = mk(0, 0, 0);
    D3 h_pos = mk(0, 0, 0), h_nrm = mk(0, 0, 0);
    int h_obj = -1;
    if constexpr (FUSE) {
      h_pos = nx_pos; h_nrm = nx_nrm; h_obj = nx_obj;
      nx_pos = mk(0, 0, 0); nx_nrm = mk(0, 0, 0); nx_obj = -1;
      if constexpr (!POOL) {
        if (__ballot(pend) != 0ull) {
          if (pend) {
            D3 so, sd;
            stash_take_ray(stash, lane, so, sd);
            double t = INF;
            D3 hn = mk(0, 0, 0);
#if RPT_PRETRACE_CULL
            const uint64_t skip = cull_skip_mask(pa.flat, near);
            PROF_COUNT(PF_P_PRETRACE);
            const int ho = flat_query<false, true, CONSTS>(sc, &fl, so, sd, -INF, t, hn, skip);
#else
            const int ho = flat_query<false, false, CONSTS>(sc, &fl, so, sd, -INF, t, hn);
#endif
            n_ext++;
            if (ho < 0) hn = env_color(sc, sd);
            stash_put_hit(stash, lane, so + t * sd, hn, ho);
            pend = false;
          }
        }
      }
    } else if constexpr (PRETRACE) {
#pragma unroll 1
      for (uint32_t pass = __ballot(pend && in_path) != 0ull ? 0u : 1u; pass < 2u; pass++) {
        const bool pre = pend, run = pend || (pass == 1u && in_path);
        if (pre) stash_swap_ray(stash, lane, o, d);
        double t = INF;
        h_nrm = mk(0, 0, 0);
        h_obj = -1;
        if (run) {
          h_obj = flat_query<false>(sc, &fl, o, d, -INF, t, h_nrm);
          n_ext++;
          if (h_obj < 0) h_nrm = env_color(sc, d);
        }
        h_pos = o + t * d;
        if (pre) {
          D3 ro, rd;
          stash_take_ray(stash, lane, ro, rd);
          stash_put_dir(stash, lane, d);
          stash_put_hit(stash, lane, h_pos, h_nrm, h_obj);
          o = ro; d = rd;
          pend = false;
        }
      }
    }
    if constexpr (POOL) {
      PROF_PHASE(PF_P_HIT);
      const bool need = !in_path || h_obj < 0;
      const uint64_t need_mask = __ballot(need);
      if (need && rpt_pool_pop_ok(rpt_pool_rank(need_mask, lane), ps.cnt)) {
        if (in_path) end_path(pa, fr, rec, fold_l, fold_u, lane, fold_st, ring, h_nrm, depth, s, p_local);
        pool_take(stash, rpt_pool_slot(ps.head, rpt_pool_rank(need_mask, lane), RPT_POOL_CAP), fr, h_pos, d, h_nrm, h_obj, p_local, s, rng);
        depth = 0;
        in_path = true;
      }
      rpt_pool_after_pop(ps.head, ps.cnt, need_mask, RPT_POOL_CAP);
      PROF_PHASE(PF_P_RAYGEN);
    } else if constexpr (PRETRACE) {
      PROF_PHASE(PF_P_HIT);
      if (in_path && h_obj < 0 && stash_valid) {
        end_path(pa, fr, rec, fold_l, fold_u, lane, fold_st, ring, h_nrm, depth, s, p_local);
        in_path = false;
      }
      if (!in_path && stash_valid) {
        stash_take_hit(stash, lane, h_pos, d, h_nrm, h_obj);
        stash_take_path(stash, lane, fr, p_local, pixel, s, s_end, rng);
        stash_valid = false;
        depth = 0;
        in_path = true;
      }
      PROF_PHASE(PF_P_RAYGEN);
    }
    if constexpr (FUSE) {
      if (in_path && h_obj < 0) {
        PROF_PHASE(PF_P_ILLUM);
        ending = true;
        A_end = h_nrm;
      } else if (in_path) {
        const D3 world_pos = h_pos, nrm = h_nrm;
        const Material& mat = fl.obj_mat[h_obj];
        const D3 wo = -normalize(d);
        const D3 color = mat.emittance * ld3(mat.color);
        D3 wl, lt, wi;
        double dist;
        bool cont;
#if RPT_SHADE_SPLIT
        CLight& lg = clight(sc, 0);
        CInst& li = cinst(sc, lg.inst);
        if (lg.kind == RPT_LIGHT_OBJECT && li.kind == RPT_SHAPE_MESH && !li.has_xf && __ballot(mat.transparent != 0) == 0ull) {
          CTree& tr = ctree(sc, li.tree);
          constexpr bool CM = CONSTS && SC_MAT, CL = CONSTS && SC_LIGHT;
          const MatConsts* mcs = CM ? mat_consts_of(&fl, h_obj) : nullptr;
          double fs;
          if constexpr (CM) {
            fs = mcs->fs;
          } else {
            const D3 mc = ld3(mat.color);
            const double f0 = pow2((mat.index - 1.0) / (mat.index + 1.0));
            const double mean = ((mc.x + mc.y) + mc.z) / 3.0;
            fs = (1.0 - mat.metallic) * f0 + mat.metallic * mean;
            fs = fs * (1.0 - 0.2) + 1.0 * 0.2;
          }
          cont = depth < fr.max_bounces;
          HitDraws dr;
          hit_draws<CM>(rng, cont, tr.num_prims, tr.sample_zone, fs, dr, mcs);
          n_sh++;
          PROF_PHASE(PF_P_DRAWS);
          D3 intensity;
          illuminate_mesh<CL>(lg, tr, sc.tris + tr.prim_base + dr.tri, world_pos, dr, intensity, wl, dist,
                              CL ? light_pdf_of(sc, &fl) : nullptr);
          double pdf;
          sample_f_opaque<CM>(mat, nrm, wo, fs, dr, wi, pdf, mcs);
          lt = mk(0, 0, 0) + cmul(bsdf_opaque<CM>(mat, nrm, wo, wl, mcs), intensity) * dot(wl, nrm);
          const D3 f = bsdf_opaque<CM>(mat, nrm, wo, wi, mcs);
          PROF_PHASE(PF_P_SHADE);
          if (cont) {
            rec_store_bsdf(rec + rec_slot(fold_st, depth, ring) * REC_FIELDS, f, 1.0 / pdf, fabs(dot(wi, nrm)));
          } else {
            wi = wl;
          }
          PROF_PHASE(PF_P_RECORD);
        } else
#endif
        {
        D3 intensity;
        illuminate(sc, clight(sc, 0), world_pos, rng, intensity, wl, dist);
        n_sh++;
        PROF_PHASE(PF_P_ILLUM);
        lt = mk(0, 0, 0) + cmul(bsdf(mat, nrm, wo, wl), intensity) * dot(wl, nrm);
        PROF_PHASE(PF_P_NEE);
        wi = wl;
        double pdf = 1.0;
        cont = depth < fr.max_bounces && sample_f(mat, nrm, wo, rng, wi, pdf);
        PROF_PHASE(PF_P_SAMPLE);
        if (cont) {
          const D3 f = bsdf(mat, nrm, wo, wi);
          PROF_PHASE(PF_P_BSDF);
          rec_store_bsdf(rec + rec_slot(fold_st, depth, ring) * REC_FIELDS, f, 1.0 / pdf, fabs(dot(wi, nrm)));
          PROF_PHASE(PF_P_RECORD);
        }
        }
        double rtb = cont ? INF : -INF, rts = INF;
        D3 rnb = mk(0, 0, 0);
        const double t_stop = fmin(dist, 1.7976931348623157e308);
        d = wi;
        const int nobj = flat_query2<CONSTS>(sc, &fl, world_pos, d, wl, t_stop, rtb, rnb, rts);
        const bool vis = rts > t_stop;
        PROF_PHASE(PF_P_FUSED);
        const D3 A = color + (vis ? lt : mk(0, 0, 0));
        if (cont) {
          double* r = rec + rec_slot(fold_st, depth, ring) * REC_FIELDS;
          r[0] = A.x; r[1] = A.y; r[2] = A.z;
          n_ext++;
          nx_pos = world_pos + rtb * d;
          nx_nrm = nobj < 0 ? env_color(sc, d) : rnb;
          nx_obj = nobj;
          depth++;
        } else {
          ending = true;
          A_end = A;
        }
        PROF_PHASE(PF_P_RECORD);
      }
    } else if (in_path) {
      double t;
      D3 nrm;
      int obj;
      if constexpr (PRETRACE) {
        obj = h_obj;
        nrm = h_nrm;
      } else {
        if constexpr (IS_FLAT) {
          t = INF;
          nrm = mk(0, 0, 0);
          if constexpr (FILTERED) obj = flat_query_filtered<false>(sc, &fl, o, d, -INF, t, nrm);
          else obj = flat_query<false>(sc, &fl, o, d, -INF, t, nrm);
        } else {
          obj = closest_hit<LDS>(sc, o, d, t, nrm, kd_ldsp);
        }
        n_ext++;
        PROF_PHASE(PF_P_HIT);
      }
      D3 A;
      bool cont = false;
      if (obj < 0) {
        if constexpr (park_on) { esc = true; A = mk(0, 0, 0); }
        else if constexpr (PRETRACE) A = nrm;
        else {
#ifdef RPT_PROF_PARK
          PROF_COUNT(PF_IK_CHILD);
#endif
          A = env_color(sc, d);
        }
        PROF_PHASE(PF_P_ILLUM);
      } else {
        D3 world_pos;
        if constexpr (PRETRACE) world_pos = h_pos;
        else world_pos = o + t * d;
        const Material* matp;
        if constexpr (IS_FLAT) matp = fl.obj_mat + obj;
        else matp = sc.materials + sc.insts[obj].material;
        const Material& mat = *matp;
        D3 wo = -normalize(d);
        D3 color = mat.emittance * ld3(mat.color);
        D3 lights = mk(0, 0, 0);
        for (int l = 0; l < sc.num_lights; l++) {
          CLight& light = clight(sc, l);
          if (light.kind == RPT_LIGHT_AMBIENT) {
            lights = lights + cmul(ld3(light.color), ld3(mat.color));
          } else {
            D3 intensity, wi;
            double dist;
            illuminate(sc, light, world_pos, rng, intensity, wi, dist);
            n_sh++;
            PROF_PHASE(PF_P_ILLUM);
            bool vis;
            if constexpr (IS_FLAT) {
              double srt = INF;
              D3 srn = mk(0, 0, 0);
              const double t_stop = fmin(dist, 1.7976931348623157e308);
              if constexpr (FILTERED) flat_query_filtered<true>(sc, &fl, world_pos, wi, t_stop, srt, srn);
              else flat_query<true>(sc, &fl, world_pos, wi, t_stop, srt, srn);
              vis = srt > t_stop;
            } else {
              vis = visible<LDS>(sc, world_pos, wi, dist, kd_ldsp);
            }
            PROF_PHASE(PF_P_VIS);
            if (vis) {
              D3 f = bsdf(mat, nrm, wo, wi);
              lights = lights + cmul(f, intensity) * dot(wi, nrm);
            }
            PROF_PHASE(PF_P_NEE);
          }
        }
        A = color + lights;
        if (depth < fr.max_bounces) {
          D3 wi;
          double pdf;
          bool some = sample_f(mat, nrm, wo, rng, wi, pdf);
          PROF_PHASE(PF_P_SAMPLE);
          if (some) {
            D3 f = bsdf(mat, nrm, wo, wi);
            PROF_PHASE(PF_P_BSDF);
            const double inv_pdf = 1.0 / pdf, abscos = fabs(dot(wi, nrm));
#ifdef RPT_PROBE_NO_RING
            probe_chk += ((A.x + A.y) + A.z) + ((f.x + f.y) + f.z) + inv_pdf + abscos;
#else
            {
              double* r = rec + rec_slot(fold_st, depth, ring) * REC_FIELDS;
              r[0] = A.x; r[1] = A.y; r[2] = A.z;
              rec_store_bsdf(r, f, inv_pdf, abscos);
            }
#endif
            o = world_pos;
            d = wi;
            depth++;
            cont = true;
            PROF_PHASE(PF_P_RECORD);
          }
        }
      }
      PROF_PHASE(PF_P_RECORD);
      ending = !cont;
      A_end = A;
    }
    if constexpr (park_on) {
      if (esc && pcnt < (uint32_t)RPT_PARK_K) {
        park_push(park, lane, pcnt, park_hd, park_recs, fold_st, ring, d, depth, s, p_local);
        esc = false; ending = false;
        s++;
        in_path = false;
      }
      bool back = pcnt != 0u && (done || ending);
      if (park_recs != 0u && in_path && !ending) back = park_recs + depth >= fr.max_bounces;
      const uint64_t c0 = __ballot((pcnt & 1u) != 0u), c1 = __ballot((pcnt & 2u) != 0u), c2 = __ballot((pcnt & 4u) != 0u);
      const uint32_t n_req = (uint32_t)__popcll(c0) + 2u * (uint32_t)__popcll(c1) + 4u * (uint32_t)__popcll(c2);
      if (__ballot(back) != 0ull || n_req >= (uint32_t)RPT_PARK_FLUSH) {
        const uint64_t below = (1ull << lane) - 1ull;
        const uint32_t first = (uint32_t)__popcll(c0 & below) + 2u * (uint32_t)__popcll(c1 & below) + 4u * (uint32_t)__popcll(c2 & below);
#pragma unroll
        for (uint32_t k = 0; k < (uint32_t)RPT_PARK_K; k++)
          if (k < pcnt) park.list[first + k] = (uint8_t)(lane | (k << 6));
        __syncthreads();
        for (uint32_t g0 = 0; g0 < n_req; g0 += 64u) {
          const uint32_t g = g0 + lane;
          if (g < n_req) {
#ifdef RPT_PROF_PARK
            PROF_COUNT(PF_IK_CHILD);
#endif
            const uint32_t e = park.list[g], owner = e & 63u, k = e >> 6;
            const D3 pd = mk(park.d[k][0][owner], park.d[k][1][owner], park.d[k][2][owner]);
            const D3 col = env_color(sc, pd);
            park.d[k][0][owner] = col.x; park.d[k][1][owner] = col.y; park.d[k][2][owner] = col.z;
          }
        }
        __syncthreads();
        for (uint32_t k = 0; __ballot(k < pcnt) != 0ull; k++) {
          if (k < pcnt)
            path_ended(pa, fr, rec, fold_l, fold_u, lane, fold_st, mk(park.d[k][0][lane], park.d[k][1][lane], park.d[k][2][lane]),
                       park.u[k][0][lane], park.u[k][1][lane], park.u[k][2][lane], park.u[k][3][lane]);
        }
        pcnt = 0u; park_hd = 0xffffffffu; park_recs = 0u;
      }
      PROF_PHASE(PF_P_ILLUM);
      if (esc) {
        park_push(park, lane, pcnt, park_hd, park_recs, fold_st, ring, d, depth, s, p_local);
        ending = false;
        s++;
        in_path = false;
      }
    }
    if (ending) {
      end_path(pa, fr, rec, fold_l, fold_u, lane, fold_st, ring, A_end, depth, s, p_local);
      s++;
      in_path = false;
    }
    PROF_PHASE(PF_P_RECORD);
    if ((fold_st & 0xffffu) != 0u) {
      PROF_COUNT(PF_P_FOLDIT);
      walker_step<PARK>(pa, fr, rec, fold_l, fold_u, lane, fold_st, ring, park_hd, probe_chk);
    }
    PROF_PHASE(PF_P_FOLD);
  }
  PROF_FLUSH();
  for (int off = 32; off > 0; off >>= 1) {
    n_ext += __shfl_down(n_ext, off);
    n_sh += __shfl_down(n_sh, off);
  }
  if (lane == 0) {
    atomicAdd(pa.ray_counters, (unsigned long long)n_ext);
    atomicAdd(pa.ray_counters + 1, (unsigned long long)n_sh);
  }
}

__global__ void __launch_bounds__(256) rpt_sum_samples(Frame fr, const double* __restrict__ lbuf, uint32_t spp, int first) {
  uint32_t p = blockIdx.x * blockDim.x + threadIdx.x;
  if (p >= fr.npix) return;
  D3 acc = first ? mk(0, 0, 0) : ld3(fr.accum + 3 * (uint64_t)p);
  const double* lb = lbuf + p;
  for (uint32_t s = 0; s < spp; s++) {
    D3 L = mk(lb[0], lb[fr.npix], lb[2 * (uint64_t)fr.npix]);
    acc = acc + L;
    lb += 3 * (uint64_t)fr.npix;
  }
  fr.accum[3 * (uint64_t)p] = acc.x;
  fr.accum[3 * (uint64_t)p + 1] = acc.y;
  fr.accum[3 * (uint64_t)p + 2] = acc.z;
}
```

rpt_amd/csrc/kernels/paths_flat.inc:

```

RPT_DEV bool cube_candidate_face(D3 o, const RcpD& rdx, const RcpD& rdy, const RcpD& rdz, double t_min, double& time,
                                 uint32_t& face) {
  double x1, x2, y1, y2, z1, z2;
  uint32_t fx = 1u, fy = 3u, fz = 5u;
  div6(-0.5 - o.x, 0.5 - o.x, rdx, -0.5 - o.y, 0.5 - o.y, rdy, -0.5 - o.z, 0.5 - o.z, rdz, x1, x2, y1, y2, z1, z2);
  if (x1 > x2) { double t = x1; x1 = x2; x2 = t; fx = 0u; }
  if (y1 > y2) { double t = y1; y1 = y2; y2 = t; fy = 2u; }
  if (z1 > z2) { double t = z1; z1 = z2; z2 = t; fz = 4u; }
  double start, end;
  uint32_t sf, ef;
  if (x1 > y1 && x1 > z1) { start = x1; sf = fx; }
  else if (y1 > z1) { start = y1; sf = fy; }
  else { start = z1; sf = fz; }
  if (x2 < y2 && x2 < z2) { end = x2; ef = fx ^ 1u; }
  else if (y2 < z2) { end = y2; ef = fy ^ 1u; }
  else { end = z2; ef = fz ^ 1u; }
  if (start > end || end < t_min) return false;
  if (start < t_min) { time = end; face = ef; }
  else { time = start; face = sf; }
  return true;
}

struct LaneTree {
  uint32_t ref_base, prim_base;
};
constexpr int FLAT_RUN = RPT_FLAT_RUN;
RPT_DEV void slab_window(double fax, double fbx, double fay, double fby, double faz, double fbz, double& b_min, double& b_max) {
  b_min = fmax(fmax(fmin(fax, fbx), fmin(fay, fby)), fmin(faz, fbz));
  b_max = fmin(fmin(fmax(fax, fbx), fmax(fay, fby)), fmax(faz, fbz));
}

template <int N>
RPT_DEV uint32_t run_slabs(const Scene& sc, int i, const double* qt, double rt, double (&m)[FLAT_RUN]) {
  static_assert(N >= 1 && N <= FLAT_RUN, "run length");
  uint32_t cand = 0;
#pragma unroll
  for (int k = 0; k < FLAT_RUN; k++) m[k] = 0.0;
#pragma unroll
  for (int k = 0; k < N; k++) {
    const uint32_t ix = cinst(sc, i + k).plane_idx;
    double fax = qt[((ix >> 0) & 15u) * 64u], fbx = qt[((ix >> 4) & 15u) * 64u];
    double fay = qt[((ix >> 8) & 15u) * 64u], fby = qt[((ix >> 12) & 15u) * 64u];
    double faz = qt[((ix >> 16) & 15u) * 64u], fbz = qt[((ix >> 20) & 15u) * 64u];
    double b_min, b_max;
    slab_window(fax, fbx, fay, fby, faz, fbz, b_min, b_max);
    double mm = fmax(b_min, EPSILON);
    if (!(mm > fmin(b_max, rt))) cand |= 1u << k;
    m[k] = mm;
  }
  return cand;
}
#define RUN_SLABS_LEN(len, ...)                                       \
  switch (len) {                                                      \
    case 1: { constexpr int LEN = 1; __VA_ARGS__; } break;            \
    case 2: { constexpr int LEN = 2; __VA_ARGS__; } break;            \
    case 3: { constexpr int LEN = 3; __VA_ARGS__; } break;            \
    case 4: { constexpr int LEN = 4; __VA_ARGS__; } break;            \
    case 5: { constexpr int LEN = 5; __VA_ARGS__; } break;            \
    default: { constexpr int LEN = FLAT_RUN; __VA_ARGS__; } break;    \
  }
#define RUN_PICK(m, k) ({ double pick_ = (m)[0]; \
  _Pragma("unroll") for (int kk_ = 1; kk_ < FLAT_RUN; kk_++) pick_ = (k) == kk_ ? (m)[kk_] : pick_; \
  pick_; })
template <bool SHADOW, bool PACKED = false>
RPT_DEV bool flat_leaf_test(const Scene& sc, const FlatLds* fl, int obj, D3 o, D3 d, double t_stop, double& rt, D3& rn) {
  const uint32_t* e = fl->obj_leaf[obj];
  LaneTree lt{e[0], e[1]};
  KdNode nd;
  nd.split = 0.0; nd.a = e[2]; nd.ib = ((PACKED ? e[3] & 0xffu : e[3]) << 2) | 3u;
  return kd_leaf<true, SHADOW>(sc, lt, sc.refs + lt.ref_base, nd, o, d, EPSILON, t_stop, rt, rn);
}
struct ObjGrid {
  double qlo[3], qscale[3];
};
template <bool SHADOW>
RPT_DEV int flat_query_filtered(const Scene& sc, const FlatLds* fl, D3 o, D3 d, double t_stop, double& rt, D3& rn) {
  int obj = -1;
  const int n = sc.num_objects;
  RcpD rwx = rcp_make(d.x), rwy = rcp_make(d.y), rwz = rcp_make(d.z);
  uint64_t cand = n >= 64 ? ~0ull : (1ull << n) - 1ull;
  {
    const double RPT_C* g = (const double RPT_C*)fl->obj_grid;
    ObjGrid gr;
    for (int k = 0; k < 3; k++) { gr.qlo[k] = g[k]; gr.qscale[k] = g[3 + k]; }
    double fax, fbx, fay, fby, faz, fbz;
    div6(g[6] - o.x, g[9] - o.x, rwx, g[7] - o.y, g[10] - o.y, rwy, g[8] - o.z, g[11] - o.z, rwz, fax, fbx, fay, fby, faz, fbz);
    double b_min, b_max;
    slab_window(fax, fbx, fay, fby, faz, fbz, b_min, b_max);
    const BoxRay br = boxray_make<true>(gr, o, d, fmax(b_min, 0.0));
    if (br.on) {
      float wl, wh;
      box_window(br, EPSILON, SHADOW ? fmin(rt, t_stop) : rt, wl, wh);
      const LeafBox RPT_C* bx = (const LeafBox RPT_C*)fl->obj_box;
      uint64_t pass = fl->obj_always;
      for (int k = 0; k < n; k++) {
        LeafBox lb;
        lb.w[0] = bx[k].w[0]; lb.w[1] = bx[k].w[1]; lb.w[2] = bx[k].w[2]; lb.w[3] = 0u;
        pass |= (leaf_box_pass(lb, br, wl, wh) ? 1ull : 0ull) << k;
      }
      cand &= pass;
    }
  }
  while (__ballot(cand != 0ull) != 0ull) {
    if (cand != 0ull) {
      PROF_COUNT(PF_P_CAND);
      const int k = __ffsll((long long)cand) - 1;
      cand &= cand - 1ull;
      const uint32_t* e = fl->obj_leaf[k];
      const uint32_t kind = (e[3] >> 8) & 0xffu;
      const bool has_xf = ((e[3] >> 16) & 1u) != 0u;
      const Inst* __restrict__ in = sc.insts + k;
      bool h = false;
      if (kind == RPT_SHAPE_MESH) {
        D3 lo = o, ld = d;
        RcpD rx = rwx, ry = rwy, rz = rwz;
        if (has_xf) {
          lo = mat4_mul(in->inv, o, 1.0);
          ld = mat4_mul(in->inv, d, 0.0);
          rx = rcp_make(ld.x); ry = rcp_make(ld.y); rz = rcp_make(ld.z);
        }
        const double* bb = fl->obox + 6 * k;
        double fax, fbx, fay, fby, faz, fbz;
        div6(bb[0] - lo.x, bb[3] - lo.x, rx, bb[1] - lo.y, bb[4] - lo.y, ry, bb[2] - lo.z, bb[5] - lo.z, rz, fax, fbx, fay, fby, faz, fbz);
        double b_min, b_max;
        slab_window(fax, fbx, fay, fby, faz, fbz, b_min, b_max);
        if (!(fmax(b_min, EPSILON) > fmin(b_max, rt))) {
          D3 nn = rn;
          h = flat_leaf_test<SHADOW, true>(sc, fl, k, lo, ld, t_stop, rt, nn);
          if (h) rn = (!SHADOW && has_xf) ? normalize(mat3_mul(in->nrm, nn)) : nn;
        }
      } else if (kind == RPT_SHAPE_PLANE) {
        D3 lo = o, ld = d;
        if (has_xf) {
          lo = mat4_mul(in->inv, o, 1.0);
          ld = mat4_mul(in->inv, d, 0.0);
        }
        h = isect_plane(in->plane, lo, ld, EPSILON, rt, rn, !SHADOW);
        if (!SHADOW && h && has_xf) rn = normalize(mat3_mul(in->nrm, rn));
      } else {
        const ChildM c = ld_child(in);
        h = isect_child(c, in, o, d, EPSILON, rt, rn, !SHADOW);
      }
      if (h) obj = k;
      if (SHADOW && rt <= t_stop) cand = 0ull;
    }
  }
  return obj;
}

#if RPT_PRETRACE_CULL
typedef unsigned short US2 __attribute__((ext_vector_type(2)));
RPT_DEV uint32_t cull_near(const FlatLayout& lay, uint32_t pix, uint32_t width) {
  const uint32_t y = pix / width, x = pix - y * width;
  const US2 xy = {(unsigned short)x, (unsigned short)y};
  uint32_t near = 0u;
  for (uint32_t j = 0; j < lay.cull_n; j++) {
    const US2 t = xy - __builtin_bit_cast(US2, lay.cull_lo[j]);
    const US2 m = __builtin_elementwise_min(t, __builtin_bit_cast(US2, lay.cull_ext[j]));
    near |= (__builtin_bit_cast(uint32_t, m) == __builtin_bit_cast(uint32_t, t) ? 1u : 0u) << j;
  }
  return near;
}
RPT_DEV uint64_t cull_skip_mask(const FlatLayout& lay, uint32_t near) {
  uint64_t skip = 0ull;
  for (uint32_t j = 0; j < lay.cull_n; j++)
    if (__ballot(((near >> j) & 1u) != 0u) == 0ull) skip |= 1ull << (lay.cull_obj[j] & 63u);
  return skip;
}
#endif

template <bool SHADOW, bool CULL = false, bool CONSTS = false>
RPT_DEV int flat_query(const Scene& sc, const FlatLds* fl, D3 o, D3 d, double t_stop, double& rt, D3& rn, uint64_t skip = 0ull) {
  int obj = -1;
  uint32_t cslot = 0;
  RcpD rwx = rcp_make(d.x), rwy = rcp_make(d.y), rwz = rcp_make(d.z);
  const int n = sc.num_objects;
  const uint32_t lane = __lane_id();
  if (fl->plane_cnt) {
    const double RPT_C* pv = (const double RPT_C*)fl->plane_vals;
    const uint32_t nx = fl->plane_cnt & 15u, ny = (fl->plane_cnt >> 4) & 15u, nz = (fl->plane_cnt >> 8) & 15u;
    for (uint32_t j = 0; j < nx; j++) fl->qtab[j * 64u + lane] = (pv[j] - o.x) / d.x;
    for (uint32_t j = 0; j < ny; j++) fl->qtab[(nx + j) * 64u + lane] = (pv[4u + j] - o.y) / d.y;
    for (uint32_t j = 0; j < nz; j++) fl->qtab[(nx + ny + j) * 64u + lane] = (pv[8u + j] - o.z) / d.z;
  }
  int i = 0;
  while (i < n) {
    CInst& in = cinst(sc, i);
    if (in.kind == RPT_SHAPE_MESH && !in.has_xf) {
      uint32_t cand = 0;
      double m[FLAT_RUN];
      int len = 0;
      if (in.plane_use) {
        len = (int)in.plane_use;
        const double* qt = fl->qtab + lane;
        RUN_SLABS_LEN(len, cand = run_slabs<LEN>(sc, i, qt, rt, m))
      } else {
#pragma unroll
      for (int k = 0; k < FLAT_RUN; k++) {
        m[k] = 0.0;
        if (len == k && i + k < n) {
          CInst& q = cinst(sc, i + k);
          if (q.kind == RPT_SHAPE_MESH && !q.has_xf) {
            double fax, fbx, fay, fby, faz, fbz;
            div6(q.bounds[0] - o.x, q.bounds[3] - o.x, rwx, q.bounds[1] - o.y, q.bounds[4] - o.y, rwy,
                 q.bounds[2] - o.z, q.bounds[5] - o.z, rwz, fax, fbx, fay, fby, faz, fbz);
            double b_min, b_max;
            slab_window(fax, fbx, fay, fby, faz, fbz, b_min, b_max);
            double mm = fmax(b_min, EPSILON);
            if (!(mm > fmin(b_max, rt))) cand |= 1u << k;
            m[k] = mm;
            len = k + 1;
          }
        }
      }
      }
      while (__ballot(cand != 0u) != 0ull) {
        if (cand != 0u) {
          PROF_COUNT(PF_P_CAND);
          int k = __ffs((int)cand) - 1;
          cand &= cand - 1u;
          const double mt = RUN_PICK(m, k);
          if (!(mt > rt)) {
            if (flat_leaf_test<SHADOW>(sc, fl, i + k, o, d, t_stop, rt, rn)) obj = i + k;
            if (SHADOW && rt <= t_stop) cand = 0u;
          }
        }
      }
      if (SHADOW && rt <= t_stop) return obj;
      i += len;
    } else if (xf_cube_pair(sc, i)) {
      if (CULL && ((skip >> i) & 3ull) == 3ull) {
        PROF_COUNT(PF_P_PRECULL);
        i += 2;
        cslot += 2u;
        continue;
      }
      CInst& in2 = cinst(sc, i + 1);
      constexpr bool TAB = CONSTS && SC_CUBE && !SHADOW;
      D3 lo1 = mat4_mul(in.inv, o, 1.0), ld1 = mat4_mul(in.inv, d, 0.0);
      D3 lo2 = mat4_mul(in2.inv, o, 1.0), ld2 = mat4_mul(in2.inv, d, 0.0);
      RcpD ax = rcp_make(ld1.x), ay = rcp_make(ld1.y), az = rcp_make(ld1.z);
      RcpD bx = rcp_make(ld2.x), by = rcp_make(ld2.y), bz = rcp_make(ld2.z);
      double t1 = 0.0, t2 = 0.0;
      D3 n1 = mk(0, 0, 0), n2 = mk(0, 0, 0);
      uint32_t f1 = 0u, f2 = 0u;
      bool c1 = TAB ? cube_candidate_face(lo1, ax, ay, az, EPSILON, t1, f1) : cube_candidate(lo1, ax, ay, az, EPSILON, t1, n1);
      bool c2 = TAB ? cube_candidate_face(lo2, bx, by, bz, EPSILON, t2, f2) : cube_candidate(lo2, bx, by, bz, EPSILON, t2, n2);
      if (c1 && t1 < rt) {
        rt = t1;
        if constexpr (TAB) rn = cube_nrm_of(fl, cslot, f1);
        else if (!SHADOW) rn = normalize(mat3_mul(in.nrm, n1));
        obj = i;
      }
      if (SHADOW && rt <= t_stop) return obj;
      if (c2 && t2 < rt) {
        rt = t2;
        if constexpr (TAB) rn = cube_nrm_of(fl, cslot + 1u, f2);
        else if (!SHADOW) rn = normalize(mat3_mul(in2.nrm, n2));
        obj = i + 1;
      }
      if (SHADOW && rt <= t_stop) return obj;
      i += 2;
      cslot += 2u;
    } else {
      if (CULL && ((skip >> i) & 1ull) != 0ull) {
        i++;
        continue;
      }
      if (isect_inst<KdFlat, SHADOW>(sc, in, o, d, rwx, rwy, rwz, EPSILON, t_stop, rt, rn, (KdFlat*)nullptr)) obj = i;
      if (SHADOW && rt <= t_stop) return obj;
      i++;
    }
  }
  return obj;
}

template <bool CONSTS_>
RPT_DEV int flat_query2(const Scene& sc, const FlatLds* fl, D3 o, D3 db, D3 ds, double t_stop, double& rtb, D3& rnb,
                        double& rts) {
  constexpr bool CONSTS = CONSTS_ && SC_CUBE;
  int obj = -1;
  uint32_t cslot = 0;
  const int n = sc.num_objects;
  const uint32_t lane = __lane_id();
  const uint32_t nx = fl->plane_cnt & 15u, ny = (fl->plane_cnt >> 4) & 15u, nz = (fl->plane_cnt >> 8) & 15u;
  const uint32_t nq = nx + ny + nz;
  {
    const double RPT_C* pv = (const double RPT_C*)fl->plane_vals;
    double* qb = fl->qtab + lane;
    double* qs = qb + nq * 64u;
    for (uint32_t j = 0; j < nx; j++) { const double a = pv[j] - o.x; qb[j * 64u] = a / db.x; qs[j * 64u] = a / ds.x; }
    for (uint32_t j = 0; j < ny; j++) {
      const double a = pv[4u + j] - o.y;
      qb[(nx + j) * 64u] = a / db.y; qs[(nx + j) * 64u] = a / ds.y;
    }
    for (uint32_t j = 0; j < nz; j++) {
      const double a = pv[8u + j] - o.z;
      qb[(nx + ny + j) * 64u] = a / db.z; qs[(nx + ny + j) * 64u] = a / ds.z;
    }
  }
  int i = 0;
  while (i < n) {
    CInst& in = cinst(sc, i);
    if (in.kind == RPT_SHAPE_MESH && !in.has_xf && in.plane_use) {
      uint32_t cb = 0, cs = 0;
      double mb[FLAT_RUN], ms[FLAT_RUN];
      const int len = (int)in.plane_use;
      const double* qtb = fl->qtab + lane;
      const double* qts = qtb + nq * 64u;
      RUN_SLABS_LEN(len, cb = run_slabs<LEN>(sc, i, qtb, rtb, mb); cs = run_slabs<LEN>(sc, i, qts, rts, ms))
      if (rts <= t_stop) cs = 0u;
      while (__ballot((cb | cs) != 0u) != 0ull) {
        PROF_COUNT(PF_P_CAND);
        if (cb != 0u) {
          const int k = __ffs((int)cb) - 1;
          cb &= cb - 1u;
          const double mt = RUN_PICK(mb, k);
          if (!(mt > rtb) && flat_leaf_test<false>(sc, fl, i + k, o, db, -INF, rtb, rnb)) obj = i + k;
        }
        if (cs != 0u) {
          const int k = __ffs((int)cs) - 1;
          cs &= cs - 1u;
          const double mt = RUN_PICK(ms, k);
          if (!(mt > rts)) {
            D3 srn = mk(0, 0, 0);
            flat_leaf_test<true>(sc, fl, i + k, o, ds, t_stop, rts, srn);
            if (rts <= t_stop) cs = 0u;
          }
        }
      }
      i += len;
    } else if (xf_cube_pair(sc, i)) {
      CInst* cu[2] = {&in, &cinst(sc, i + 1)};
#pragma unroll
      for (int c = 0; c < 2; c++) {
        const CInst& q = *cu[c];
        const D3 lo = mat4_mul(q.inv, o, 1.0);
        const D3 lb = mat4_mul(q.inv, db, 0.0), ls = mat4_mul(q.inv, ds, 0.0);
        const RcpD bx = rcp_make(lb.x), by = rcp_make(lb.y), bz = rcp_make(lb.z);
        const RcpD sx = rcp_make(ls.x), sy = rcp_make(ls.y), sz = rcp_make(ls.z);
        double tb = 0.0, ts = 0.0;
        D3 nb = mk(0, 0, 0), ns = mk(0, 0, 0);
        uint32_t fb = 0u;
        const bool hb = CONSTS ? cube_candidate_face(lo, bx, by, bz, EPSILON, tb, fb) : cube_candidate(lo, bx, by, bz, EPSILON, tb, nb);
        const bool hs = cube_candidate(lo, sx, sy, sz, EPSILON, ts, ns);
        if (hb && tb < rtb) {
          rtb = tb;
          if constexpr (CONSTS) rnb = cube_nrm_of(fl, cslot + (uint32_t)c, fb);
          else rnb = normalize(mat3_mul(q.nrm, nb));
          obj = i + c;
        }
        if (hs && ts < rts) rts = ts;
      }
      i += 2;
      cslot += 2u;
    } else {
      if (!(rtb == -INF)) {
        const RcpD rx = rcp_make(db.x), ry = rcp_make(db.y), rz = rcp_make(db.z);
        if (isect_inst<KdFlat, false>(sc, in, o, db, rx, ry, rz, EPSILON, -INF, rtb, rnb, (KdFlat*)nullptr)) obj = i;
      }
      if (!(rts <= t_stop)) {
        const RcpD rx = rcp_make(ds.x), ry = rcp_make(ds.y), rz = rcp_make(ds.z);
        D3 srn = mk(0, 0, 0);
        isect_inst<KdFlat, true>(sc, in, o, ds, rx, ry, rz, EPSILON, t_stop, rts, srn, (KdFlat*)nullptr);
      }
      i++;
    }
  }
  return obj;
}
```

rpt_amd/csrc/kernels/paths_shade.inc:

```

#if RPT_SHADE_SPLIT
struct HitDraws {
  uint64_t tri;
  uint64_t a, b;
  uint64_t th;
  uint64_t qa, qb;
  bool spec;
};
template <bool CONSTS = false>
RPT_DEV void hit_draws(Rng& r, bool sf, uint64_t n, uint64_t zone, double f, HitDraws& o, const MatConsts* mc = nullptr) {
  o.tri = gen_index_zone(r, n, zone);
  next2_u64(r, o.a, o.b);
  while ((o.a >> 11) + (o.b >> 11) >= (1ull << 53) + 2ull) {
    PROF_COUNT(PF_P_REJECT);
    next2_u64(r, o.a, o.b);
  }
  o.th = 1ull << 63; o.qa = 0; o.qb = 0; o.spec = false;
  if (!sf) return;
  if constexpr (CONSTS) o.spec = f == 1.0 ? true : next_u64(r) < mc->p_int;
  else o.spec = gen_bool(r, f);
  if (o.spec) o.th = next_u64(r);
  for (;;) {
    PROF_COUNT(PF_P_REJECT);
    next2_u64(r, o.qa, o.qb);
    const double x = u52_of(o.qa) * 2.0 + -1.0, y = u52_of(o.qb) * 2.0 + -1.0;
    const double sum = x * x + y * y;
    if (o.spec ? sum < 1.0 : sum <= 1.0) break;
  }
}

template <bool CONSTS = false>
RPT_DEV D3 bsdf_opaque(const Material& m, D3 n, D3 wo, D3 wi, const MatConsts* mc = nullptr) {
  D3 color = ld3(m.color);
  double n_dot_wi = dot(n, wi);
  double n_dot_wo = dot(n, wo);
  const bool lit = !__builtin_signbit(n_dot_wi) && !__builtin_signbit(n_dot_wo);
  const D3 one = mk(1, 1, 1);
  double m2, m2pi;
  D3 f0, omf0;
  if constexpr (CONSTS) {
    m2 = mc->m2; m2pi = mc->m2pi;
    f0 = ld3(mc->f0); omf0 = ld3(mc->omf0);
  } else {
    m2 = m.roughness * m.roughness;
    m2pi = m2 * PI;
    double f0s = pow2((m.index - 1.0) / (m.index + 1.0));
    f0 = lerp(mk(f0s, f0s, f0s), color, m.metallic);
    omf0 = one - f0;
  }
  D3 h = normalize(wi + wo);
  double wo_dot_h = dot(wo, h);
  double n_dot_h = dot(n, h);
  double nh2 = pow2(n_dot_h);
  double dd = rptc_exp((nh2 - 1.0) / (m2 * nh2)) / (m2pi * nh2 * nh2);
  D3 f = f0 + omf0 * pow5(1.0 - wo_dot_h);
  double ga = n_dot_wi * n_dot_h, gb = n_dot_wo * n_dot_h;
  double g = fmin(ga, gb);
  g = (2.0 * g) / wo_dot_h;
  g = fmin(g, 1.0);
  D3 q = dd * f * g / (4.0 * n_dot_wo * n_dot_wi);
  D3 diffuse = cmul(one - f, color) / PI;
  return lit ? q + diffuse : mk(0, 0, 0);
}

template <bool CONSTS = false>
RPT_DEV void sample_f_opaque(const Material& m, D3 n, D3 wo, double f, const HitDraws& dr, D3& wi, double& pdf,
                             const MatConsts* mc = nullptr) {
  double m2;
  if constexpr (CONSTS) m2 = mc->m2;
  else m2 = m.roughness * m.roughness;
  const double u_theta = (double)(dr.th >> 11) * (1.0 / 9007199254740992.0);
  const double x = u52_of(dr.qa) * 2.0 + -1.0, y = u52_of(dr.qb) * 2.0 + -1.0;
  const double sum = x * x + y * y;
  double theta = rptc_atan(sqrt(m2 * -rpt_log(u_theta)));
  double sin_t, cos_t;
  rptc_sincos_pio2(theta, &sin_t, &cos_t);
  double diff = x * x - y * y;
  double cx = diff / sum, cy = 2.0 * x * y / sum;
  const D3 loc = dr.spec ? mk(cx * sin_t, cy * sin_t, cos_t) : mk(x, y, sqrt(1.0 - x * x - y * y));
  const D3 world = local_to_world_mul(n, loc);
  wi = dr.spec ? -(wo - world * (dot(world, wo) * 2.0)) : world;
  double p = 0.0;
  {
    D3 h = normalize(wi + wo);
    double p_h;
    if constexpr (CONSTS) {
      double cos_t = fabs(dot(h, n));
      double sin_t = sqrt(1.0 - cos_t * cos_t);
      p_h = (1.0 / (mc->m2pi * pow3(cos_t))) * rptc_exp(-pow2(sin_t / cos_t) / m2);
    } else {
      p_h = beckmann_pdf(m2, n, h);
    }
    p += f * p_h / (4.0 * fabs(dot(h, wo)));
  }
  p += (1.0 - f) * fmax(dot(wi, n), 0.0) * FRAC_1_PI;
  pdf = p;
}

template <bool CONSTS = false>
RPT_DEV void illuminate_mesh(CLight& l, CTree& tr, const Tri* __restrict__ tp, D3 pos, const HitDraws& dr, D3& intensity,
                             D3& wi, double& dist, const double* light_pdf = nullptr) {
  const double u = (double)(dr.a >> 11) * (1.0 / 9007199254740992.0), v = (double)(dr.b >> 11) * (1.0 / 9007199254740992.0);
  double w = 1.0 - u - v;
  D3 v1 = ld3(tp->v), v2 = ld3(tp->v + 3), v3 = ld3(tp->v + 6);
  D3 n1 = ld3(tp->v + 9), n2 = ld3(tp->v + 12), n3 = ld3(tp->v + 15);
  SampleOut s{u * v1 + v * v2 + w * v3, normalize(u * n1 + v * n2 + w * n3), 0.0};
  if constexpr (CONSTS) {
    s.p = light_pdf[dr.tri];
  } else {
    double area = 0.5 * length(cross(v2 - v1, v3 - v1));
    s.p = 1.0 / area;
    s.p = s.p / (double)tr.num_prims;
  }
  D3 disp = s.v - pos;
  double len = length(disp);
  double cosine = fmax(-dot(disp, s.n), 0.0) / len;
  double surface_area = fmax(cosine, 0.0) / (len * len);
  intensity = ld3(l.mat_color) * l.mat_emittance * surface_area / s.p;
  wi = disp / len;
  dist = len;
}
#endif
```

rpt_amd/csrc/kernels/shapes.inc:

```


RPT_DEV bool isect_sphere(D3 o, D3 d, double t_min, double& rt, D3& rn, const bool want_n = true) {
  double a = length2(d);
  double b = dot(d, o);
  double c = length2(o) - 1.0;
  double disc = b * b - a * c;
  if (__builtin_signbit(disc)) return false;
  disc = sqrt(disc);
  RcpD ra = rcp_make(a);
  double t = div_r(-b - disc, ra);
  if (t < t_min) {
    t = div_r(-b + disc, ra);
    if (t < t_min) return false;
  }
  if (t < rt) {
    rt = t;
    if (want_n) rn = normalize(o + t * d);
    return true;
  }
  return false;
}

template <class P> RPT_DEV bool isect_plane(P pl, D3 o, D3 d, double t_min, double& rt, D3& rn, const bool want_n = true) {
  D3 n = ld3(pl);
  double cosine = dot(n, d);
  if (fabs(cosine) < 1e-8) return false;
  double time = (pl[3] - dot(n, o)) / cosine;
  if (time >= t_min && time < rt) {
    rt = time;
    if (want_n) rn = (-normalize(n)) * signum(cosine);
    return true;
  }
  return false;
}

RPT_DEV bool cube_candidate(D3 o, const RcpD& rdx, const RcpD& rdy, const RcpD& rdz, double t_min, double& time,
                            D3& normal) {
  double x1, x2, y1, y2, z1, z2, sx = -1.0, sy = -1.0, sz = -1.0;
  div6(-0.5 - o.x, 0.5 - o.x, rdx, -0.5 - o.y, 0.5 - o.y, rdy, -0.5 - o.z, 0.5 - o.z, rdz, x1, x2, y1, y2, z1, z2);
  if (x1 > x2) { double t = x1; x1 = x2; x2 = t; sx = 1.0; }
  if (y1 > y2) { double t = y1; y1 = y2; y2 = t; sy = 1.0; }
  if (z1 > z2) { double t = z1; z1 = z2; z2 = t; sz = 1.0; }
  double start, end;
  D3 sn, en;
  if (x1 > y1 && x1 > z1) { start = x1; sn = mk(sx, 0, 0); }
  else if (y1 > z1) { start = y1; sn = mk(0, sy, 0); }
  else { start = z1; sn = mk(0, 0, sz); }
  if (x2 < y2 && x2 < z2) { end = x2; en = mk(-sx, 0, 0); }
  else if (y2 < z2) { end = y2; en = mk(0, -sy, 0); }
  else { end = z2; en = mk(0, 0, -sz); }
  if (start > end || end < t_min) return false;
  if (start < t_min) { time = end; normal = en; }
  else { time = start; normal = sn; }
  return true;
}
RPT_DEV bool isect_cube(D3 o, const RcpD& rdx, const RcpD& rdy, const RcpD& rdz, double t_min, double& rt,
                        D3& rn) {
  double time = 0.0;
  D3 normal = mk(0, 0, 0);
  if (cube_candidate(o, rdx, rdy, rdz, t_min, time, normal) && time < rt) {
    rt = time;
    rn = normal;
    return true;
  }
  return false;
}

#ifdef RPT_EXT_SHAPES
RPT_DEV bool isect_monomial(double height, D3 o, D3 d, const RcpD& rdx, const RcpD& rdy, const RcpD& rdz,
                            double t_min, double& rt, D3& rn, const bool want_n) {
  double x1, x2, y1, y2, z1, z2;
  div6(-1.0 - o.x, 1.0 - o.x, rdx, 0.0 - o.y, height - o.y, rdy, -1.0 - o.z, 1.0 - o.z, rdz, x1, x2, y1, y2, z1, z2);
  double b_min = fmax(fmax(fmin(x1, x2), fmin(y1, y2)), fmin(z1, z2));
  double b_max = fmin(fmin(fmax(x1, x2), fmax(y1, y2)), fmax(z1, z2));
  if (fmax(b_min, t_min) > fmin(b_max, rt)) return false;
  auto dist = [&](double t) {
    double x = o.x + t * d.x, y = o.y + t * d.y, z = o.z + t * d.z;
    double s = x * x + z * z;
    return y - height * (s * s);
  };
  double t_max;
  const bool maximize = dist(t_min) < 0.0;
  if (maximize) {
    double coef0 = o.x * o.x + o.z * o.z;
    double coef1 = 2. * (o.x * d.x + o.z * d.z);
    double coef2 = d.x * d.x + d.z * d.z;
    double cur_x = (b_min + b_max) / 2.;
    for (int i = 0; i < 10; i++) {
      double f = dist(cur_x);
      if (f > 0.) break;
      double t = cur_x;
      double dy1 = 2. * coef0 * coef1 + 2. * t * (coef1 * coef1 + 2. * coef0 * coef2)
                   + 3. * (t * t) * 2. * coef1 * coef2 + 4. * (t * (t * t)) * coef2 * coef2;
      double der = d.y - height * dy1;
      double dy2 = 2. * (coef1 * coef1 + 2. * coef0 * coef2) + 3. * 2. * t * 2. * coef1 * coef2
                   + 4. * 3. * (t * t) * coef2 * coef2;
      double der2 = -height * dy2;
      cur_x -= der / der2;
    }
    t_max = cur_x;
    if (t_max < t_min) return false;
  } else {
    t_max = 10000.;
  }
  if ((dist(t_min) < 0.0) == (dist(t_max) < 0.0)) return false;
  double l = t_min, r = t_max;
#pragma unroll 1
  for (int i = 0; i < 60; i++) {
    double m = (l + r) / 2.0;
    if ((dist(m) >= 0.0) == maximize) r = m;
    else l = m;
  }
  if (r > rt) return false;
  D3 pos = o + r * d;
  double s = pos.x * pos.x + pos.z * pos.z;
  if (s > 1.0) return false;
  rt = r;
  if (want_n) {
    D3 n = normalize(mk(height * 4.0 * pos.x * s, -1.0, height * 4.0 * pos.z * s));
    if (dot(n, d) > 0.0) n = -n;
    rn = n;
  }
  return true;
}

#endif

struct TriPlane {
  double cosine, time;
};
RPT_DEV TriPlane tri_plane(const TriX* __restrict__ tx, D3 o, D3 d) {
  D3 pn = ld3(tx->pn), v1 = ld3(tx->v1);
  TriPlane r;
  r.cosine = dot(pn, d);
  r.time = dot(pn, v1 - o) / r.cosine;
  return r;
}
struct TriBary {
  double u, v, w;
};
RPT_DEV TriBary tri_bary(const TriX* __restrict__ tx, TriPlane pl, D3 o, D3 d) {
  D3 v1 = ld3(tx->v1), d0 = ld3(tx->d0), d1 = ld3(tx->d1);
  D3 d2 = (o + pl.time * d) - v1;
  double d00 = tx->d00, d01 = tx->d01, d11 = tx->d11, denom = tx->denom;
  double d20 = dot(d2, d0);
  double d21 = dot(d2, d1);
  TriBary b;
  b.v = (d11 * d20 - d01 * d21) / denom;
  b.w = (d00 * d21 - d01 * d20) / denom;
  b.u = 1.0 - b.v - b.w;
  return b;
}
RPT_DEV bool tri_accept(const TriX* __restrict__ tx, const Tri* __restrict__ tris, const uint32_t* __restrict__ refp,
                        TriPlane pl, D3 o, D3 d, double t_min, double& rt, D3& rn, const bool want_n) {
  const double time = pl.time;
  if ((fabs(pl.cosine) < 1e-8) | (time < t_min) | (time >= rt)) return false;
  D3 v1 = ld3(tx->v1), d0 = ld3(tx->d0), d1 = ld3(tx->d1);
  D3 d2 = (o + time * d) - v1;
  double d00 = tx->d00, d01 = tx->d01, d11 = tx->d11, denom = tx->denom;
  double d20 = dot(d2, d0);
  double d21 = dot(d2, d1);
  double v = (d11 * d20 - d01 * d21) / denom;
  double w = (d00 * d21 - d01 * d20) / denom;
  double u = 1.0 - v - w;
  if ((u >= 0.0) & (v >= 0.0) & (w >= 0.0)) {
    rt = time;
    if (want_n) {
      const Tri* tp = tris + *refp;
      D3 n1 = ld3(tp->v + 9), n2 = ld3(tp->v + 12), n3 = ld3(tp->v + 15);
      rn = normalize(u * n1 + v * n2 + w * n3);
    }
    return true;
  }
  return false;
}

struct ChildM {
  double m[16];
  int32_t kind, has_xf;
};
RPT_DEV ChildM ld_child(const Inst* __restrict__ in) {
  ChildM c;
  c.kind = in->kind;
  c.has_xf = in->has_xf;
#pragma unroll
  for (int col = 0; col < 4; col++)
#pragma unroll
    for (int r = 0; r < 3; r++) c.m[4 * col + r] = in->inv[4 * col + r];
  return c;
}
RPT_DEV bool isect_child(const ChildM& c, const Inst* __restrict__ in, D3 o, D3 d, double t_min, double& rt, D3& rn,
                         const bool want_n) {
  D3 lo = o, ld = d;
  if (c.has_xf) {
    lo = mat4_mul(c.m, o, 1.0);
    ld = mat4_mul(c.m, d, 0.0);
  }
  bool hit;
  if (c.kind == RPT_SHAPE_SPHERE) {
    hit = isect_sphere(lo, ld, t_min, rt, rn, want_n);
  } else {
    RcpD rx = rcp_make(ld.x), ry = rcp_make(ld.y), rz = rcp_make(ld.z);
#ifdef RPT_EXT_SHAPES
    if (c.kind == RPT_SHAPE_MONOMIAL) hit = isect_monomial(in->plane[0], lo, ld, rx, ry, rz, t_min, rt, rn, want_n);
    else
#endif
      hit = isect_cube(lo, rx, ry, rz, t_min, rt, rn);
  }
  if (want_n && hit && c.has_xf) rn = normalize(mat3_mul(in->nrm, rn));
  return hit;
}

template <bool SHADOW>
RPT_DEV bool tri_batch(const TriX* __restrict__ recs, const Tri* __restrict__ tris, const uint32_t* __restrict__ refp,
                       uint32_t m, bool pair_only, D3 o, D3 d, double t_min, double& rt, D3& rn) {
  bool found = false, h;
  TriPlane p0 = tri_plane(recs, o, d);
  TriPlane p1 = tri_plane(recs + (m > 1 ? 1u : 0u), o, d);
  if (pair_only) {
    if (m > 1) {
      TriBary b0 = tri_bary(recs, p0, o, d), b1 = tri_bary(recs + 1, p1, o, d);
      int win = -1;
      if (!(fabs(p0.cosine) < 1e-8) && !(p0.time < t_min || p0.time >= rt) && b0.u >= 0.0 && b0.v >= 0.0 && b0.w >= 0.0) {
        rt = p0.time;
        win = 0;
      }
      if (!(fabs(p1.cosine) < 1e-8) && !(p1.time < t_min || p1.time >= rt) && b1.u >= 0.0 && b1.v >= 0.0 && b1.w >= 0.0) {
        rt = p1.time;
        win = 1;
      }
      if (win >= 0 && !SHADOW) {
        const Tri* tp = tris + refp[win];
        TriBary b = win ? b1 : b0;
        D3 n1 = ld3(tp->v + 9), n2 = ld3(tp->v + 12), n3 = ld3(tp->v + 15);
        rn = normalize(b.u * n1 + b.v * n2 + b.w * n3);
      }
      return win >= 0;
    }
    return tri_accept(recs, tris, refp, p0, o, d, t_min, rt, rn, !SHADOW);
  }
  TriPlane p2 = tri_plane(recs + (m > 2 ? 2u : 0u), o, d);
  TriPlane p3 = tri_plane(recs + (m > 3 ? 3u : 0u), o, d);
  h = tri_accept(recs, tris, refp, p0, o, d, t_min, rt, rn, !SHADOW);
  found = found || h;
  if (m > 1) { h = tri_accept(recs + 1, tris, refp + 1, p1, o, d, t_min, rt, rn, !SHADOW); found = found || h; }
  if (m > 2) { h = tri_accept(recs + 2, tris, refp + 2, p2, o, d, t_min, rt, rn, !SHADOW); found = found || h; }
  if (m > 3) { h = tri_accept(recs + 3, tris, refp + 3, p3, o, d, t_min, rt, rn, !SHADOW); found = found || h; }
  return found;
}

struct BoxRay {
  float ax, ay, az, bx, by, bz;
  double t0;
  bool on;
};
constexpr double BOX_PAR = 1e30;
template <bool QUADRIC, class TreeT> RPT_DEV BoxRay boxray_make(const TreeT& tr, D3 o, D3 d, double t0) {
  constexpr double FAR = QUADRIC ? 1e7 : 1e12;
  BoxRay r;
  const bool zx = d.x == 0.0, zy = d.y == 0.0, zz = d.z == 0.0;
  double rx = 1.0 / d.x, ry = 1.0 / d.y, rz = 1.0 / d.z;
  double gx = 0.0, gy = 0.0, gz = 0.0;
  if (zx || zy || zz) {
    gx = (o.x - tr.qlo[0]) / tr.qscale[0]; gy = (o.y - tr.qlo[1]) / tr.qscale[1]; gz = (o.z - tr.qlo[2]) / tr.qscale[2];
  }
  double ax = zx ? BOX_PAR : tr.qscale[0] * rx, ay = zy ? BOX_PAR : tr.qscale[1] * ry, az = zz ? BOX_PAR : tr.qscale[2] * rz;
  const double ux = (tr.qlo[0] - o.x) * rx, uy = (tr.qlo[1] - o.y) * ry, uz = (tr.qlo[2] - o.z) * rz;
  double bx = zx ? -gx * BOX_PAR : ux - t0, by = zy ? -gy * BOX_PAR : uy - t0, bz = zz ? -gz * BOX_PAR : uz - t0;
  const bool okx = zx ? fabs(gx) < 1e6 : (fabs(ax) > 1e-30 && fabs(ax) < 1e30 && fabs(bx) < 1e6 * fabs(ax) && fabs(ux) < FAR * fabs(ax));
  const bool oky = zy ? fabs(gy) < 1e6 : (fabs(ay) > 1e-30 && fabs(ay) < 1e30 && fabs(by) < 1e6 * fabs(ay) && fabs(uy) < FAR * fabs(ay));
  const bool okz = zz ? fabs(gz) < 1e6 : (fabs(az) > 1e-30 && fabs(az) < 1e30 && fabs(bz) < 1e6 * fabs(az) && fabs(uz) < FAR * fabs(az));
  r.on = !(zx && zy && zz) && okx && oky && okz && fabs(t0) < 1e300;
  r.ax = (float)ax; r.ay = (float)ay; r.az = (float)az;
  r.bx = (float)bx; r.by = (float)by; r.bz = (float)bz;
  r.t0 = t0;
  return r;
}
RPT_DEV void box_window(const BoxRay& r, double t_lo, double t_hi, float& wl, float& wh) {
  float l = (float)(t_lo - r.t0), h = (float)(t_hi - r.t0);
  wl = l - (fabsf(l) * 1.2e-7f + 1e-30f);
  wh = h + (fabsf(h) * 1.2e-7f + 1e-30f);
}
typedef float F2 __attribute__((ext_vector_type(2)));
RPT_DEV bool leaf_box_pass(const LeafBox& lb, const BoxRay& r, float wl, float wh) {
  const float cx = (float)(lb.w[0] & 0xffffu), cy = (float)(lb.w[1] & 0xffffu), cz = (float)(lb.w[2] & 0xffffu);
  const float ex = (float)(lb.w[0] >> 16), ey = (float)(lb.w[1] >> 16), ez = (float)(lb.w[2] >> 16);
  const float tx = __builtin_fmaf(cx, r.ax, r.bx), ty = __builtin_fmaf(cy, r.ay, r.by), tz = __builtin_fmaf(cz, r.az, r.bz);
  const float hx = fabsf(r.ax), hy = fabsf(r.ay), hz = fabsf(r.az);
  const F2 X = __builtin_elementwise_fma(F2{ex, ex}, F2{-hx, hx}, F2{tx, tx});
  const F2 Y = __builtin_elementwise_fma(F2{ey, ey}, F2{-hy, hy}, F2{ty, ty});
  const F2 Z = __builtin_elementwise_fma(F2{ez, ez}, F2{-hz, hz}, F2{tz, tz});
  const float lo = fmaxf(fmaxf(X.x, Y.x), Z.x), hi = fminf(fminf(X.y, Y.y), Z.y);
  return lo <= hi && !(hi < wl) && !(lo > wh);
}

template <bool SHADOW, class TreeT>
RPT_DEV bool kd_leaf_boxed(const Scene& sc, const TreeT& tr, const uint32_t* __restrict__ refs, KdNode n, D3 o, D3 d,
                           double t_min, double t_stop, double& rt, D3& rn, const BoxRay& br) {
  bool found = false;
  const uint32_t first = n.a, cnt = n.ib >> 2;
  const TriX* __restrict__ recs = sc.lrec + tr.ref_base + first;
  const LeafBox* __restrict__ boxes = sc.lbox + tr.ref_base + first;
  const Tri* __restrict__ tris = sc.tris + tr.prim_base;
  for (uint32_t base = 0; base < cnt; base += 32u) {
    const uint32_t lim = min(cnt - base, 32u);
    uint32_t m = lim >= 32u ? 0xffffffffu : ((1u << lim) - 1u);
    if (br.on) {
      float wl, wh;
      box_window(br, t_min, SHADOW ? fmin(rt, t_stop) : rt, wl, wh);
      m = 0u;
#ifndef RPT_BOX_BATCH
#define RPT_BOX_BATCH 8
#endif
      for (uint32_t b = 0; b < lim; b += RPT_BOX_BATCH) {
        PROF_COUNT(PF_TT_BOX);
        LeafBox w[RPT_BOX_BATCH];
#pragma unroll
        for (uint32_t k = 0; k < RPT_BOX_BATCH; k++) w[k] = boxes[base + min(b + k, lim - 1u)];
        uint32_t p = 0u;
#pragma unroll
        for (uint32_t k = 0; k < RPT_BOX_BATCH; k++) p |= (leaf_box_pass(w[k], br, wl, wh) ? 1u : 0u) << k;
        m |= p << b;
      }
      m &= lim >= 32u ? 0xffffffffu : ((1u << lim) - 1u);
    }
    PROF_PHASE(PF_TT_BOX);
    while (m) {
      PROF_COUNT(PF_TT_EXACT);
      const uint32_t i = (uint32_t)__ffs((int)m) - 1u;
      m &= m - 1u;
      const uint32_t j = base + i;
      TriPlane p = tri_plane(recs + j, o, d);
      bool h = tri_accept(recs + j, tris, refs + first + j, p, o, d, t_min, rt, rn, !SHADOW);
      found = found || h;
      if (SHADOW && rt <= t_stop) break;
    }
    PROF_PHASE(PF_TT_EXACT);
    if (SHADOW && rt <= t_stop) return found;
  }
  return found;
}

struct KdNoLds;

template <bool TRIS, bool SHADOW, class TreeT>
RPT_DEV bool kd_leaf(const Scene& sc, const TreeT& tr, const uint32_t* __restrict__ refs, KdNode n, D3 o, D3 d,
                     double t_min, double t_stop, double& rt, D3& rn, const BoxRay* br = nullptr) {
  bool found = false;
  uint32_t first = n.a, cnt = n.ib >> 2;
  if (br && br->on && cnt > 2u) {
    if constexpr (TRIS) {
      return kd_leaf_boxed<SHADOW>(sc, tr, refs, n, o, d, t_min, t_stop, rt, rn, *br);
    } else {
      const LeafBox* __restrict__ boxes = sc.lbox + tr.ref_base + first;
      const Inst* __restrict__ kids = sc.insts + tr.prim_base;
      for (uint32_t base = 0; base < cnt; base += 32u) {
        const uint32_t lim = min(cnt - base, 32u);
        float wl, wh;
        box_window(*br, t_min, SHADOW ? fmin(rt, t_stop) : rt, wl, wh);
        uint32_t m = 0u;
#ifndef RPT_GBOX_BATCH
#define RPT_GBOX_BATCH 4
#endif
        for (uint32_t b = 0; b < lim; b += RPT_GBOX_BATCH) {
          PROF_COUNT(PF_IK_BOX);
          LeafBox w[RPT_GBOX_BATCH];
#pragma unroll
          for (uint32_t k = 0; k < RPT_GBOX_BATCH; k++) w[k] = boxes[base + b + k];
          uint32_t p = 0u;
#pragma unroll
          for (uint32_t k = 0; k < RPT_GBOX_BATCH; k++) p |= (leaf_box_pass(w[k], *br, wl, wh) ? 1u : 0u) << k;
          m |= p << b;
        }
        m &= lim >= 32u ? 0xffffffffu : ((1u << lim) - 1u);
        while (m) {
          PROF_COUNT(PF_IK_CHILD);
          const uint32_t i = (uint32_t)__ffs((int)m) - 1u;
          m &= m - 1u;
          const Inst* __restrict__ c = kids + refs[first + base + i];
          ChildM cur = ld_child(c);
          bool h = isect_child(cur, c, o, d, t_min, rt, rn, !SHADOW);
          found = found || h;
          if (SHADOW && rt <= t_stop) return found;
        }
      }
      return found;
    }
  }
  if (TRIS) {
    const TriX* __restrict__ recs = sc.lrec + tr.ref_base + first;
    const Tri* __restrict__ tris = sc.tris + tr.prim_base;
    for (uint32_t b = 0; b < cnt; b += 4) {
      PROF_COUNT(PF_IK_TRI);
      bool h = tri_batch<SHADOW>(recs + b, tris, refs + first + b, cnt - b, cnt <= 2, o, d, t_min, rt, rn);
      found = found || h;
      if (SHADOW && rt <= t_stop) break;
    }
  } else {
    if (cnt == 0) return false;
    const Inst* __restrict__ base = sc.insts + tr.prim_base;
    const Inst* __restrict__ c = base + refs[first];
    ChildM cur = ld_child(c);
    for (uint32_t i = 0; i < cnt; i++) {
      PROF_COUNT(PF_IK_CHILD);
      const Inst* __restrict__ cn = c;
      ChildM nx = cur;
      if (i + 1 < cnt) {
        cn = base + refs[first + i + 1];
        nx = ld_child(cn);
      }
      bool h = isect_child(cur, c, o, d, t_min, rt, rn, !SHADOW);
      found = found || h;
      if (SHADOW && rt <= t_stop) break;
      c = cn;
      cur = nx;
    }
  }
  return found;
}
```

rpt_amd/csrc/kernels/vec.inc:

```

struct D3 {
  double x, y, z;
};
RPT_DEV D3 mk(double x, double y, double z) { return D3{x, y, z}; }
RPT_DEV D3 operator+(D3 a, D3 b) { return {a.x + b.x, a.y + b.y, a.z + b.z}; }
RPT_DEV D3 operator-(D3 a, D3 b) { return {a.x - b.x, a.y - b.y, a.z - b.z}; }
RPT_DEV D3 operator-(D3 a) { return {-a.x, -a.y, -a.z}; }
RPT_DEV D3 operator*(double s, D3 a) { return {s * a.x, s * a.y, s * a.z}; }
RPT_DEV D3 operator*(D3 a, double s) { return {a.x * s, a.y * s, a.z * s}; }

struct RcpD {
  double d, r;
  bool ok;
};
RPT_DEV bool safe_exp(double x) {
  uint32_t e = ((uint32_t)(__double_as_longlong(x) >> 52)) & 0x7ffu;
  return e - 623u < 800u;
}
RPT_DEV RcpD rcp_make(double d) {
  RcpD o;
  o.d = d;
  o.ok = safe_exp(d);
  double x = __builtin_amdgcn_rcp(d);
  double e0 = __builtin_fma(-d, x, 1.0);
  double r1 = __builtin_fma(x, e0, x);
  double e1 = __builtin_fma(-d, r1, 1.0);
  o.r = __builtin_fma(r1, e1, r1);
  return o;
}
RPT_DEV double div_fast(double n, const RcpD& rc) {
  double q = n * rc.r;
  double e = __builtin_fma(-rc.d, q, n);
  return __builtin_fma(e, rc.r, q);
}
RPT_DEV bool safe_range(double mn, double mx) { return mn >= 0x1p-400 && mx < 0x1p400; }
RPT_DEV bool safe_coord(double x) {
  uint32_t e = ((uint32_t)(__double_as_longlong(x) >> 52)) & 0x7ffu;
  return x == 0.0 || e - 683u < 739u;
}
RPT_DEV double fmin_raw(double a, double b) { double r; asm("v_min_f64 %0, %1, %2" : "=v"(r) : "v"(a), "v"(b)); return r; }
RPT_DEV double fmax_raw(double a, double b) { double r; asm("v_max_f64 %0, %1, %2" : "=v"(r) : "v"(a), "v"(b)); return r; }
RPT_DEV double div_r(double n, const RcpD& rc) { return n / rc.d; }
RPT_DEV void div6(double n0, double n1, const RcpD& rx, double n2, double n3, const RcpD& ry, double n4, double n5,
                  const RcpD& rz, double& q0, double& q1, double& q2, double& q3, double& q4, double& q5) {
  q0 = div_r(n0, rx); q1 = div_r(n1, rx);
  q2 = div_r(n2, ry); q3 = div_r(n3, ry);
  q4 = div_r(n4, rz); q5 = div_r(n5, rz);
}
RPT_DEV D3 operator/(D3 a, double s) {
  RcpD rc = rcp_make(s);
  return {div_r(a.x, rc), div_r(a.y, rc), div_r(a.z, rc)};
}
RPT_DEV D3 cmul(D3 a, D3 b) { return {a.x * b.x, a.y * b.y, a.z * b.z}; }
RPT_DEV double dot(D3 a, D3 b) { return (a.x * b.x + a.y * b.y) + a.z * b.z; }
RPT_DEV double length2(D3 a) { return dot(a, a); }
RPT_DEV double length(D3 a) { return sqrt(dot(a, a)); }
RPT_DEV D3 normalize(D3 a) { return a / length(a); }
RPT_DEV D3 cross(D3 a, D3 b) {
  return {a.y * b.z - a.z * b.y, a.z * b.x - a.x * b.z, a.x * b.y - a.y * b.x};
}
template <class P> RPT_DEV D3 ld3(P p) { return {p[0], p[1], p[2]}; }
RPT_DEV double sel(int axis, D3 v) { return axis == 0 ? v.x : (axis == 1 ? v.y : v.z); }
RPT_DEV double signum(double x) { return x != x ? x : (__builtin_signbit(x) ? -1.0 : 1.0); }
RPT_DEV bool is_normal(double x) { return __builtin_isnormal(x); }
RPT_DEV double pow2(double x) { return x * x; }
RPT_DEV double pow3(double x) { return x * (x * x); }
RPT_DEV double pow5(double x) { double x2 = x * x; return x * (x2 * x2); }
RPT_DEV D3 lerp(D3 a, D3 b, double t) { return a * (1.0 - t) + b * t; }

template <class P> RPT_DEV D3 mat4_mul(P m, D3 v, double w) {
  D3 r;
  r.x = ((m[0] * v.x + m[4] * v.y) + m[8] * v.z) + m[12] * w;
  r.y = ((m[1] * v.x + m[5] * v.y) + m[9] * v.z) + m[13] * w;
  r.z = ((m[2] * v.x + m[6] * v.y) + m[10] * v.z) + m[14] * w;
  return r;
}
template <class P> RPT_DEV D3 mat3_mul(P m, D3 v) {
  D3 r;
  r.x = (m[0] * v.x + m[3] * v.y) + m[6] * v.z;
  r.y = (m[1] * v.x + m[4] * v.y) + m[7] * v.z;
  r.z = (m[2] * v.x + m[5] * v.y) + m[8] * v.z;
  return r;
}
```

Before: 1641.

## Batch independent IEEE f64 divisions to interleave their expansion sequences

Adds div_ieee<N>, which expands N independent double divisions into the div_scale/rcp/fma/div_fmas/div_fixup sequence stage by stage, so the dependent chains of several divisions interleave instead of running back to back. This batching is applied to slab tests, plane quotient tables, triangle plane and barycentric solves, normalisation, BRDF evaluation and light sampling on the traced and shaded paths, behind RPT_DIV_BATCH (default on). It is meant to cut latency stalls from serial f64 division, at the cost of higher register pressure that may lower occupancy. It also adds eval_math modes for benchmarking batched division.

```diff
diff --git a/rpt_amd/csrc/api_render.cpp b/rpt_amd/csrc/api_render.cpp
--- a/rpt_amd/csrc/api_render.cpp
+++ b/rpt_amd/csrc/api_render.cpp
@@ -627,7 +627,7 @@
 }
 
 int rptgpu_eval_math(rptgpu_scene* h, int fn, uint64_t n, const double* x, const double* y, double* out) {
-  if (!h || (n && (!x || !out)) || fn < 0 || fn > 7 || (fn >= 6 && n && !y))
+  if (!h || (n && (!x || !out)) || fn < 0 || fn > 11 || (fn >= 6 && n && !y))
     return fail(h, RPTGPU_E_INVALID_ARGUMENT, "bad argument");
   if (!n) return RPTGPU_OK;
   return guarded(h, h->device, [&]() -> int {
diff --git a/rpt_amd/csrc/kernels.h b/rpt_amd/csrc/kernels.h
--- a/rpt_amd/csrc/kernels.h
+++ b/rpt_amd/csrc/kernels.h
@@ -40,6 +40,9 @@
 #endif
 #ifndef RPT_POOL_REFILL
 #define RPT_POOL_REFILL 56u
+#endif
+#ifndef RPT_DIV_BATCH
+#define RPT_DIV_BATCH 1
 #endif
 #define RPT_PATHS_POOL_LDS (RPT_POOL_CAP * 100u)
 static_assert(RPT_POOL_CAP >= 64u && RPT_POOL_REFILL >= 1u && RPT_POOL_REFILL <= RPT_POOL_CAP,
diff --git a/rpt_amd/csrc/kernels/buffer.inc b/rpt_amd/csrc/kernels/buffer.inc
--- a/rpt_amd/csrc/kernels/buffer.inc
+++ b/rpt_amd/csrc/kernels/buffer.inc
@@ -134,6 +134,24 @@
   out[p] = ss / ((double)nb - 1.0);
 }
 
+template <int N> RPT_DEV void eval_div_batch(uint64_t i, uint64_t n, const double* x, const double* y, double* out) {
+  const uint64_t t = n / N;
+  if (i < t) {
+    uint64_t p[N];
+    double nn[N], dd[N], q[N];
+#pragma unroll
+    for (int s = 0; s < N; s++) {
+      p[s] = (uint64_t)s * t + (i + (uint64_t)s * 4099ull) % t;
+      nn[s] = y[p[s]];
+      dd[s] = x[p[s]];
+    }
+    div_ieee<N>(nn, dd, q);
+#pragma unroll
+    for (int s = 0; s < N; s++) out[p[s]] = q[s];
+  }
+  if (i < n - t * N) out[t * N + i] = y[t * N + i] / x[t * N + i];
+}
+
 __global__ void __launch_bounds__(256) rpt_eval_math(int fn, uint64_t n, const double* __restrict__ x,
                                                      const double* __restrict__ y, double* __restrict__ out) {
   uint64_t i = (uint64_t)blockIdx.x * blockDim.x + threadIdx.x;
@@ -147,6 +165,10 @@
     case 4: rptc_sincos_pio2(x[i], &s, &c); out[i] = c; break;
     case 5: out[i] = rptc_acos(x[i]); break;
     case 6: out[i] = rptc_atan2(y[i], x[i]); break;
+    case 8: eval_div_batch<2>(i, n, x, y, out); break;
+    case 9: eval_div_batch<3>(i, n, x, y, out); break;
+    case 10: eval_div_batch<4>(i, n, x, y, out); break;
+    case 11: eval_div_batch<6>(i, n, x, y, out); break;
     default: {
       RcpD rc = rcp_make(x[i]);
       double a = fabs(y[i]);
diff --git a/rpt_amd/csrc/kernels/paths.inc b/rpt_amd/csrc/kernels/paths.inc
--- a/rpt_amd/csrc/kernels/paths.inc
+++ b/rpt_amd/csrc/kernels/paths.inc
@@ -560,7 +560,7 @@
       } else if (in_path) {
         const D3 world_pos = h_pos, nrm = h_nrm;
         const Material& mat = fl.obj_mat[h_obj];
-        const D3 wo = -normalize(d);
+        const D3 wo = -normalize_b(d);
         const D3 color = mat.emittance * ld3(mat.color);
         D3 wl, lt, wi;
         double dist;
diff --git a/rpt_amd/csrc/kernels/paths_flat.inc b/rpt_amd/csrc/kernels/paths_flat.inc
--- a/rpt_amd/csrc/kernels/paths_flat.inc
+++ b/rpt_amd/csrc/kernels/paths_flat.inc
@@ -3,7 +3,7 @@
                                  uint32_t& face) {
   double x1, x2, y1, y2, z1, z2;
   uint32_t fx = 1u, fy = 3u, fz = 5u;
-  div6(-0.5 - o.x, 0.5 - o.x, rdx, -0.5 - o.y, 0.5 - o.y, rdy, -0.5 - o.z, 0.5 - o.z, rdz, x1, x2, y1, y2, z1, z2);
+  div6<true>(-0.5 - o.x, 0.5 - o.x, rdx, -0.5 - o.y, 0.5 - o.y, rdy, -0.5 - o.z, 0.5 - o.z, rdz, x1, x2, y1, y2, z1, z2);
   if (x1 > x2) { double t = x1; x1 = x2; x2 = t; fx = 0u; }
   if (y1 > y2) { double t = y1; y1 = y2; y2 = t; fy = 2u; }
   if (z1 > z2) { double t = z1; z1 = z2; z2 = t; fz = 4u; }
@@ -62,13 +62,13 @@
 #define RUN_PICK(m, k) ({ double pick_ = (m)[0]; \
   _Pragma("unroll") for (int kk_ = 1; kk_ < FLAT_RUN; kk_++) pick_ = (k) == kk_ ? (m)[kk_] : pick_; \
   pick_; })
-template <bool SHADOW, bool PACKED = false>
+template <bool SHADOW, bool PACKED = false, bool DIVB = false>
 RPT_DEV bool flat_leaf_test(const Scene& sc, const FlatLds* fl, int obj, D3 o, D3 d, double t_stop, double& rt, D3& rn) {
   const uint32_t* e = fl->obj_leaf[obj];
   LaneTree lt{e[0], e[1]};
   KdNode nd;
   nd.split = 0.0; nd.a = e[2]; nd.ib = ((PACKED ? e[3] & 0xffu : e[3]) << 2) | 3u;
-  return kd_leaf<true, SHADOW>(sc, lt, sc.refs + lt.ref_base, nd, o, d, EPSILON, t_stop, rt, rn);
+  return kd_leaf<true, SHADOW, DIVB>(sc, lt, sc.refs + lt.ref_base, nd, o, d, EPSILON, t_stop, rt, rn);
 }
 struct ObjGrid {
   double qlo[3], qscale[3];
@@ -169,7 +169,36 @@
 }
 #endif
 
-template <bool SHADOW, bool CULL = false, bool CONSTS = false>
+RPT_DEV void plane_quotients(const double RPT_C* pv, uint32_t cnt, double o, double d, double* q) {
+  uint32_t j = 0;
+  for (; j + 2u <= cnt; j += 2u) {
+    const double n2[2] = {pv[j] - o, pv[j + 1u] - o}, d2[2] = {d, d};
+    double t[2];
+    div_ieee<2>(n2, d2, t);
+    q[j * 64u] = t[0]; q[(j + 1u) * 64u] = t[1];
+  }
+  for (; j < cnt; j++) q[j * 64u] = (pv[j] - o) / d;
+}
+RPT_DEV void plane_quotients2(const double RPT_C* pv, uint32_t cnt, double o, double db, double ds, double* qb, double* qs) {
+  uint32_t j = 0;
+  for (; j + 2u <= cnt; j += 2u) {
+    const double a0 = pv[j] - o, a1 = pv[j + 1u] - o;
+    const double n4[4] = {a0, a0, a1, a1}, d4[4] = {db, ds, db, ds};
+    double t[4];
+    div_ieee<4>(n4, d4, t);
+    qb[j * 64u] = t[0]; qs[j * 64u] = t[1];
+    qb[(j + 1u) * 64u] = t[2]; qs[(j + 1u) * 64u] = t[3];
+  }
+  for (; j < cnt; j++) {
+    const double a = pv[j] - o;
+    const double n2[2] = {a, a}, d2[2] = {db, ds};
+    double t[2];
+    div_ieee<2>(n2, d2, t);
+    qb[j * 64u] = t[0]; qs[j * 64u] = t[1];
+  }
+}
+
+template <bool SHADOW, bool CULL = false, bool CONSTS = false, bool DIVB = CULL || CONSTS>
 RPT_DEV int flat_query(const Scene& sc, const FlatLds* fl, D3 o, D3 d, double t_stop, double& rt, D3& rn, uint64_t skip = 0ull) {
   int obj = -1;
   uint32_t cslot = 0;
@@ -179,9 +208,16 @@
   if (fl->plane_cnt) {
     const double RPT_C* pv = (const double RPT_C*)fl->plane_vals;
     const uint32_t nx = fl->plane_cnt & 15u, ny = (fl->plane_cnt >> 4) & 15u, nz = (fl->plane_cnt >> 8) & 15u;
-    for (uint32_t j = 0; j < nx; j++) fl->qtab[j * 64u + lane] = (pv[j] - o.x) / d.x;
-    for (uint32_t j = 0; j < ny; j++) fl->qtab[(nx + j) * 64u + lane] = (pv[4u + j] - o.y) / d.y;
-    for (uint32_t j = 0; j < nz; j++) fl->qtab[(nx + ny + j) * 64u + lane] = (pv[8u + j] - o.z) / d.z;
+    if constexpr (DIVB && RPT_DIV_BATCH != 0) {
+      double* q = fl->qtab + lane;
+      plane_quotients(pv, nx, o.x, d.x, q);
+      plane_quotients(pv + 4, ny, o.y, d.y, q + nx * 64u);
+      plane_quotients(pv + 8, nz, o.z, d.z, q + (nx + ny) * 64u);
+    } else {
+      for (uint32_t j = 0; j < nx; j++) fl->qtab[j * 64u + lane] = (pv[j] - o.x) / d.x;
+      for (uint32_t j = 0; j < ny; j++) fl->qtab[(nx + j) * 64u + lane] = (pv[4u + j] - o.y) / d.y;
+      for (uint32_t j = 0; j < nz; j++) fl->qtab[(nx + ny + j) * 64u + lane] = (pv[8u + j] - o.z) / d.z;
+    }
   }
   int i = 0;
   while (i < n) {
@@ -202,7 +238,7 @@
           CInst& q = cinst(sc, i + k);
           if (q.kind == RPT_SHAPE_MESH && !q.has_xf) {
             double fax, fbx, fay, fby, faz, fbz;
-            div6(q.bounds[0] - o.x, q.bounds[3] - o.x, rwx, q.bounds[1] - o.y, q.bounds[4] - o.y, rwy,
+            div6<DIVB>(q.bounds[0] - o.x, q.bounds[3] - o.x, rwx, q.bounds[1] - o.y, q.bounds[4] - o.y, rwy,
                  q.bounds[2] - o.z, q.bounds[5] - o.z, rwz, fax, fbx, fay, fby, faz, fbz);
             double b_min, b_max;
             slab_window(fax, fbx, fay, fby, faz, fbz, b_min, b_max);
@@ -221,7 +257,7 @@
           cand &= cand - 1u;
           const double mt = RUN_PICK(m, k);
           if (!(mt > rt)) {
-            if (flat_leaf_test<SHADOW>(sc, fl, i + k, o, d, t_stop, rt, rn)) obj = i + k;
+            if (flat_leaf_test<SHADOW, false, DIVB>(sc, fl, i + k, o, d, t_stop, rt, rn)) obj = i + k;
             if (SHADOW && rt <= t_stop) cand = 0u;
           }
         }
@@ -244,19 +280,19 @@
       double t1 = 0.0, t2 = 0.0;
       D3 n1 = mk(0, 0, 0), n2 = mk(0, 0, 0);
       uint32_t f1 = 0u, f2 = 0u;
-      bool c1 = TAB ? cube_candidate_face(lo1, ax, ay, az, EPSILON, t1, f1) : cube_candidate(lo1, ax, ay, az, EPSILON, t1, n1);
-      bool c2 = TAB ? cube_candidate_face(lo2, bx, by, bz, EPSILON, t2, f2) : cube_candidate(lo2, bx, by, bz, EPSILON, t2, n2);
+      bool c1 = TAB ? cube_candidate_face(lo1, ax, ay, az, EPSILON, t1, f1) : cube_candidate<DIVB>(lo1, ax, ay, az, EPSILON, t1, n1);
+      bool c2 = TAB ? cube_candidate_face(lo2, bx, by, bz, EPSILON, t2, f2) : cube_candidate<DIVB>(lo2, bx, by, bz, EPSILON, t2, n2);
       if (c1 && t1 < rt) {
         rt = t1;
         if constexpr (TAB) rn = cube_nrm_of(fl, cslot, f1);
-        else if (!SHADOW) rn = normalize(mat3_mul(in.nrm, n1));
+        else if (!SHADOW) rn = normalize_t<DIVB>(mat3_mul(in.nrm, n1));
         obj = i;
       }
       if (SHADOW && rt <= t_stop) return obj;
       if (c2 && t2 < rt) {
         rt = t2;
         if constexpr (TAB) rn = cube_nrm_of(fl, cslot + 1u, f2);
-        else if (!SHADOW) rn = normalize(mat3_mul(in2.nrm, n2));
+        else if (!SHADOW) rn = normalize_t<DIVB>(mat3_mul(in2.nrm, n2));
         obj = i + 1;
       }
       if (SHADOW && rt <= t_stop) return obj;
@@ -289,6 +325,11 @@
     const double RPT_C* pv = (const double RPT_C*)fl->plane_vals;
     double* qb = fl->qtab + lane;
     double* qs = qb + nq * 64u;
+#if RPT_DIV_BATCH
+    plane_quotients2(pv, nx, o.x, db.x, ds.x, qb, qs);
+    plane_quotients2(pv + 4, ny, o.y, db.y, ds.y, qb + nx * 64u, qs + nx * 64u);
+    plane_quotients2(pv + 8, nz, o.z, db.z, ds.z, qb + (nx + ny) * 64u, qs + (nx + ny) * 64u);
+#else
     for (uint32_t j = 0; j < nx; j++) { const double a = pv[j] - o.x; qb[j * 64u] = a / db.x; qs[j * 64u] = a / ds.x; }
     for (uint32_t j = 0; j < ny; j++) {
       const double a = pv[4u + j] - o.y;
@@ -298,6 +339,7 @@
       const double a = pv[8u + j] - o.z;
       qb[(nx + ny + j) * 64u] = a / db.z; qs[(nx + ny + j) * 64u] = a / ds.z;
     }
+#endif
   }
   int i = 0;
   while (i < n) {
@@ -316,7 +358,7 @@
           const int k = __ffs((int)cb) - 1;
           cb &= cb - 1u;
           const double mt = RUN_PICK(mb, k);
-          if (!(mt > rtb) && flat_leaf_test<false>(sc, fl, i + k, o, db, -INF, rtb, rnb)) obj = i + k;
+          if (!(mt > rtb) && flat_leaf_test<false, false, true>(sc, fl, i + k, o, db, -INF, rtb, rnb)) obj = i + k;
         }
         if (cs != 0u) {
           const int k = __ffs((int)cs) - 1;
@@ -324,7 +366,7 @@
           const double mt = RUN_PICK(ms, k);
           if (!(mt > rts)) {
             D3 srn = mk(0, 0, 0);
-            flat_leaf_test<true>(sc, fl, i + k, o, ds, t_stop, rts, srn);
+            flat_leaf_test<true, false, true>(sc, fl, i + k, o, ds, t_stop, rts, srn);
             if (rts <= t_stop) cs = 0u;
           }
         }
@@ -342,12 +384,12 @@
         double tb = 0.0, ts = 0.0;
         D3 nb = mk(0, 0, 0), ns = mk(0, 0, 0);
         uint32_t fb = 0u;
-        const bool hb = CONSTS ? cube_candidate_face(lo, bx, by, bz, EPSILON, tb, fb) : cube_candidate(lo, bx, by, bz, EPSILON, tb, nb);
-        const bool hs = cube_candidate(lo, sx, sy, sz, EPSILON, ts, ns);
+        const bool hb = CONSTS ? cube_candidate_face(lo, bx, by, bz, EPSILON, tb, fb) : cube_candidate<true>(lo, bx, by, bz, EPSILON, tb, nb);
+        const bool hs = cube_candidate<true>(lo, sx, sy, sz, EPSILON, ts, ns);
         if (hb && tb < rtb) {
           rtb = tb;
           if constexpr (CONSTS) rnb = cube_nrm_of(fl, cslot + (uint32_t)c, fb);
-          else rnb = normalize(mat3_mul(q.nrm, nb));
+          else rnb = normalize_b(mat3_mul(q.nrm, nb));
           obj = i + c;
         }
         if (hs && ts < rts) rts = ts;
diff --git a/rpt_amd/csrc/kernels/paths_shade.inc b/rpt_amd/csrc/kernels/paths_shade.inc
--- a/rpt_amd/csrc/kernels/paths_shade.inc
+++ b/rpt_amd/csrc/kernels/paths_shade.inc
@@ -48,18 +48,29 @@
     f0 = lerp(mk(f0s, f0s, f0s), color, m.metallic);
     omf0 = one - f0;
   }
-  D3 h = normalize(wi + wo);
+  D3 h = normalize_b(wi + wo);
   double wo_dot_h = dot(wo, h);
   double n_dot_h = dot(n, h);
   double nh2 = pow2(n_dot_h);
+#if RPT_DIV_BATCH
+  double ga = n_dot_wi * n_dot_h, gb = n_dot_wo * n_dot_h;
+  double g = fmin(ga, gb);
+  const double sn[2] = {nh2 - 1.0, 2.0 * g}, sd[2] = {m2 * nh2, wo_dot_h};
+  double sq[2];
+  div_ieee<2>(sn, sd, sq);
+  double dd = rptc_exp(sq[0]) / (m2pi * nh2 * nh2);
+  D3 f = f0 + omf0 * pow5(1.0 - wo_dot_h);
+  g = sq[1];
+#else
   double dd = rptc_exp((nh2 - 1.0) / (m2 * nh2)) / (m2pi * nh2 * nh2);
   D3 f = f0 + omf0 * pow5(1.0 - wo_dot_h);
   double ga = n_dot_wi * n_dot_h, gb = n_dot_wo * n_dot_h;
   double g = fmin(ga, gb);
   g = (2.0 * g) / wo_dot_h;
+#endif
   g = fmin(g, 1.0);
-  D3 q = dd * f * g / (4.0 * n_dot_wo * n_dot_wi);
-  D3 diffuse = cmul(one - f, color) / PI;
+  D3 q = div3(dd * f * g, 4.0 * n_dot_wo * n_dot_wi);
+  D3 diffuse = div3(cmul(one - f, color), PI);
   return lit ? q + diffuse : mk(0, 0, 0);
 }
 
@@ -76,13 +87,16 @@
   double sin_t, cos_t;
   rptc_sincos_pio2(theta, &sin_t, &cos_t);
   double diff = x * x - y * y;
-  double cx = diff / sum, cy = 2.0 * x * y / sum;
+  const double cn[2] = {diff, 2.0 * x * y}, cd[2] = {sum, sum};
+  double cq[2];
+  div_ieee<2>(cn, cd, cq);
+  const double cx = cq[0], cy = cq[1];
   const D3 loc = dr.spec ? mk(cx * sin_t, cy * sin_t, cos_t) : mk(x, y, sqrt(1.0 - x * x - y * y));
   const D3 world = local_to_world_mul(n, loc);
   wi = dr.spec ? -(wo - world * (dot(world, wo) * 2.0)) : world;
   double p = 0.0;
   {
-    D3 h = normalize(wi + wo);
+    D3 h = normalize_b(wi + wo);
     double p_h;
     if constexpr (CONSTS) {
       double cos_t = fabs(dot(h, n));
@@ -104,7 +118,7 @@
   double w = 1.0 - u - v;
   D3 v1 = ld3(tp->v), v2 = ld3(tp->v + 3), v3 = ld3(tp->v + 6);
   D3 n1 = ld3(tp->v + 9), n2 = ld3(tp->v + 12), n3 = ld3(tp->v + 15);
-  SampleOut s{u * v1 + v * v2 + w * v3, normalize(u * n1 + v * n2 + w * n3), 0.0};
+  SampleOut s{u * v1 + v * v2 + w * v3, normalize_b(u * n1 + v * n2 + w * n3), 0.0};
   if constexpr (CONSTS) {
     s.p = light_pdf[dr.tri];
   } else {
@@ -114,10 +128,20 @@
   }
   D3 disp = s.v - pos;
   double len = length(disp);
+#if RPT_DIV_BATCH
+  const double ln[4] = {fmax(-dot(disp, s.n), 0.0), disp.x, disp.y, disp.z}, ld[4] = {len, len, len, len};
+  double lq[4];
+  div_ieee<4>(ln, ld, lq);
+  double cosine = lq[0];
+  double surface_area = fmax(cosine, 0.0) / (len * len);
+  intensity = div3(ld3(l.mat_color) * l.mat_emittance * surface_area, s.p);
+  wi = mk(lq[1], lq[2], lq[3]);
+#else
   double cosine = fmax(-dot(disp, s.n), 0.0) / len;
   double surface_area = fmax(cosine, 0.0) / (len * len);
   intensity = ld3(l.mat_color) * l.mat_emittance * surface_area / s.p;
   wi = disp / len;
+#endif
   dist = len;
 }
 #endif
diff --git a/rpt_amd/csrc/kernels/shapes.inc b/rpt_amd/csrc/kernels/shapes.inc
--- a/rpt_amd/csrc/kernels/shapes.inc
+++ b/rpt_amd/csrc/kernels/shapes.inc
@@ -34,10 +34,11 @@
   return false;
 }
 
+template <bool DIVB = false>
 RPT_DEV bool cube_candidate(D3 o, const RcpD& rdx, const RcpD& rdy, const RcpD& rdz, double t_min, double& time,
                             D3& normal) {
   double x1, x2, y1, y2, z1, z2, sx = -1.0, sy = -1.0, sz = -1.0;
-  div6(-0.5 - o.x, 0.5 - o.x, rdx, -0.5 - o.y, 0.5 - o.y, rdy, -0.5 - o.z, 0.5 - o.z, rdz, x1, x2, y1, y2, z1, z2);
+  div6<DIVB>(-0.5 - o.x, 0.5 - o.x, rdx, -0.5 - o.y, 0.5 - o.y, rdy, -0.5 - o.z, 0.5 - o.z, rdz, x1, x2, y1, y2, z1, z2);
   if (x1 > x2) { double t = x1; x1 = x2; x2 = t; sx = 1.0; }
   if (y1 > y2) { double t = y1; y1 = y2; y2 = t; sy = 1.0; }
   if (z1 > z2) { double t = z1; z1 = z2; z2 = t; sz = 1.0; }
@@ -151,6 +152,37 @@
   b.u = 1.0 - b.v - b.w;
   return b;
 }
+RPT_DEV void tri_plane2(const TriX* __restrict__ ta, const TriX* __restrict__ tb, D3 o, D3 d, TriPlane& pa, TriPlane& pb) {
+  D3 pna = ld3(ta->pn), v1a = ld3(ta->v1), pnb = ld3(tb->pn), v1b = ld3(tb->v1);
+  pa.cosine = dot(pna, d);
+  pb.cosine = dot(pnb, d);
+  const double n[2] = {dot(pna, v1a - o), dot(pnb, v1b - o)}, c[2] = {pa.cosine, pb.cosine};
+  double t[2];
+  div_ieee<2>(n, c, t);
+  pa.time = t[0];
+  pb.time = t[1];
+}
+RPT_DEV void tri_bary2(const TriX* __restrict__ ta, TriPlane pa, const TriX* __restrict__ tb, TriPlane pb, D3 o, D3 d,
+                       TriBary& ba, TriBary& bb) {
+  double n[4], c[4], q[4];
+  const TriX* __restrict__ tx[2] = {ta, tb};
+  const double time[2] = {pa.time, pb.time};
+#pragma unroll
+  for (int k = 0; k < 2; k++) {
+    D3 v1 = ld3(tx[k]->v1), d0 = ld3(tx[k]->d0), d1 = ld3(tx[k]->d1);
+    D3 d2 = (o + time[k] * d) - v1;
+    double d00 = tx[k]->d00, d01 = tx[k]->d01, d11 = tx[k]->d11;
+    double d20 = dot(d2, d0);
+    double d21 = dot(d2, d1);
+    n[2 * k] = d11 * d20 - d01 * d21;
+    n[2 * k + 1] = d00 * d21 - d01 * d20;
+    c[2 * k] = c[2 * k + 1] = tx[k]->denom;
+  }
+  div_ieee<4>(n, c, q);
+  ba.v = q[0]; ba.w = q[1]; ba.u = 1.0 - ba.v - ba.w;
+  bb.v = q[2]; bb.w = q[3]; bb.u = 1.0 - bb.v - bb.w;
+}
+template <bool DIVB = false>
 RPT_DEV bool tri_accept(const TriX* __restrict__ tx, const Tri* __restrict__ tris, const uint32_t* __restrict__ refp,
                         TriPlane pl, D3 o, D3 d, double t_min, double& rt, D3& rn, const bool want_n) {
   const double time = pl.time;
@@ -160,15 +192,24 @@
   double d00 = tx->d00, d01 = tx->d01, d11 = tx->d11, denom = tx->denom;
   double d20 = dot(d2, d0);
   double d21 = dot(d2, d1);
-  double v = (d11 * d20 - d01 * d21) / denom;
-  double w = (d00 * d21 - d01 * d20) / denom;
+  double v, w;
+  if constexpr (DIVB) {
+    const double bn[2] = {d11 * d20 - d01 * d21, d00 * d21 - d01 * d20}, bd[2] = {denom, denom};
+    double bq[2];
+    div_ieee<2>(bn, bd, bq);
+    v = bq[0];
+    w = bq[1];
+  } else {
+    v = (d11 * d20 - d01 * d21) / denom;
+    w = (d00 * d21 - d01 * d20) / denom;
+  }
   double u = 1.0 - v - w;
   if ((u >= 0.0) & (v >= 0.0) & (w >= 0.0)) {
     rt = time;
     if (want_n) {
       const Tri* tp = tris + *refp;
       D3 n1 = ld3(tp->v + 9), n2 = ld3(tp->v + 12), n3 = ld3(tp->v + 15);
-      rn = normalize(u * n1 + v * n2 + w * n3);
+      rn = normalize_t<DIVB>(u * n1 + v * n2 + w * n3);
     }
     return true;
   }
@@ -211,15 +252,27 @@
   return hit;
 }
 
-template <bool SHADOW>
+template <bool SHADOW, bool DIVB_ = false>
 RPT_DEV bool tri_batch(const TriX* __restrict__ recs, const Tri* __restrict__ tris, const uint32_t* __restrict__ refp,
                        uint32_t m, bool pair_only, D3 o, D3 d, double t_min, double& rt, D3& rn) {
+  constexpr bool DIVB = DIVB_ && RPT_DIV_BATCH != 0;
   bool found = false, h;
-  TriPlane p0 = tri_plane(recs, o, d);
-  TriPlane p1 = tri_plane(recs + (m > 1 ? 1u : 0u), o, d);
+  TriPlane p0, p1;
+  if constexpr (DIVB) {
+    tri_plane2(recs, recs + (m > 1 ? 1u : 0u), o, d, p0, p1);
+  } else {
+    p0 = tri_plane(recs, o, d);
+    p1 = tri_plane(recs + (m > 1 ? 1u : 0u), o, d);
+  }
   if (pair_only) {
     if (m > 1) {
-      TriBary b0 = tri_bary(recs, p0, o, d), b1 = tri_bary(recs + 1, p1, o, d);
+      TriBary b0, b1;
+      if constexpr (DIVB) {
+        tri_bary2(recs, p0, recs + 1, p1, o, d, b0, b1);
+      } else {
+        b0 = tri_bary(recs, p0, o, d);
+        b1 = tri_bary(recs + 1, p1, o, d);
+      }
       int win = -1;
       if (!(fabs(p0.cosine) < 1e-8) && !(p0.time < t_min || p0.time >= rt) && b0.u >= 0.0 && b0.v >= 0.0 && b0.w >= 0.0) {
         rt = p0.time;
@@ -233,19 +286,24 @@
         const Tri* tp = tris + refp[win];
         TriBary b = win ? b1 : b0;
         D3 n1 = ld3(tp->v + 9), n2 = ld3(tp->v + 12), n3 = ld3(tp->v + 15);
-        rn = normalize(b.u * n1 + b.v * n2 + b.w * n3);
+        rn = normalize_t<DIVB>(b.u * n1 + b.v * n2 + b.w * n3);
       }
       return win >= 0;
     }
-    return tri_accept(recs, tris, refp, p0, o, d, t_min, rt, rn, !SHADOW);
-  }
-  TriPlane p2 = tri_plane(recs + (m > 2 ? 2u : 0u), o, d);
-  TriPlane p3 = tri_plane(recs + (m > 3 ? 3u : 0u), o, d);
-  h = tri_accept(recs, tris, refp, p0, o, d, t_min, rt, rn, !SHADOW);
+    return tri_accept<DIVB>(recs, tris, refp, p0, o, d, t_min, rt, rn, !SHADOW);
+  }
+  TriPlane p2, p3;
+  if constexpr (DIVB) {
+    tri_plane2(recs + (m > 2 ? 2u : 0u), recs + (m > 3 ? 3u : 0u), o, d, p2, p3);
+  } else {
+    p2 = tri_plane(recs + (m > 2 ? 2u : 0u), o, d);
+    p3 = tri_plane(recs + (m > 3 ? 3u : 0u), o, d);
+  }
+  h = tri_accept<DIVB>(recs, tris, refp, p0, o, d, t_min, rt, rn, !SHADOW);
   found = found || h;
-  if (m > 1) { h = tri_accept(recs + 1, tris, refp + 1, p1, o, d, t_min, rt, rn, !SHADOW); found = found || h; }
-  if (m > 2) { h = tri_accept(recs + 2, tris, refp + 2, p2, o, d, t_min, rt, rn, !SHADOW); found = found || h; }
-  if (m > 3) { h = tri_accept(recs + 3, tris, refp + 3, p3, o, d, t_min, rt, rn, !SHADOW); found = found || h; }
+  if (m > 1) { h = tri_accept<DIVB>(recs + 1, tris, refp + 1, p1, o, d, t_min, rt, rn, !SHADOW); found = found || h; }
+  if (m > 2) { h = tri_accept<DIVB>(recs + 2, tris, refp + 2, p2, o, d, t_min, rt, rn, !SHADOW); found = found || h; }
+  if (m > 3) { h = tri_accept<DIVB>(recs + 3, tris, refp + 3, p3, o, d, t_min, rt, rn, !SHADOW); found = found || h; }
   return found;
 }
 
@@ -343,7 +401,7 @@
 
 struct KdNoLds;
 
-template <bool TRIS, bool SHADOW, class TreeT>
+template <bool TRIS, bool SHADOW, bool DIVB = false , class TreeT>
 RPT_DEV bool kd_leaf(const Scene& sc, const TreeT& tr, const uint32_t* __restrict__ refs, KdNode n, D3 o, D3 d,
                      double t_min, double t_stop, double& rt, D3& rn, const BoxRay* br = nullptr) {
   bool found = false;
@@ -392,7 +450,7 @@
     const Tri* __restrict__ tris = sc.tris + tr.prim_base;
     for (uint32_t b = 0; b < cnt; b += 4) {
       PROF_COUNT(PF_IK_TRI);
-      bool h = tri_batch<SHADOW>(recs + b, tris, refs + first + b, cnt - b, cnt <= 2, o, d, t_min, rt, rn);
+      bool h = tri_batch<SHADOW, DIVB>(recs + b, tris, refs + first + b, cnt - b, cnt <= 2, o, d, t_min, rt, rn);
       found = found || h;
       if (SHADOW && rt <= t_stop) break;
     }
diff --git a/rpt_amd/csrc/kernels/vec.inc b/rpt_amd/csrc/kernels/vec.inc
--- a/rpt_amd/csrc/kernels/vec.inc
+++ b/rpt_amd/csrc/kernels/vec.inc
@@ -41,21 +41,71 @@
 RPT_DEV double fmin_raw(double a, double b) { double r; asm("v_min_f64 %0, %1, %2" : "=v"(r) : "v"(a), "v"(b)); return r; }
 RPT_DEV double fmax_raw(double a, double b) { double r; asm("v_max_f64 %0, %1, %2" : "=v"(r) : "v"(a), "v"(b)); return r; }
 RPT_DEV double div_r(double n, const RcpD& rc) { return n / rc.d; }
+template <int N> RPT_DEV void div_ieee(const double (&n)[N], const double (&d)[N], double (&q)[N]) {
+#if RPT_DIV_BATCH
+  double ds[N], ns[N], r[N], e[N], m[N];
+  bool f[N], f0;
+#pragma unroll
+  for (int k = 0; k < N; k++) ds[k] = __builtin_amdgcn_div_scale(n[k], d[k], false, &f0);
+#pragma unroll
+  for (int k = 0; k < N; k++) r[k] = __builtin_amdgcn_rcp(ds[k]);
+#pragma unroll
+  for (int k = 0; k < N; k++) e[k] = __builtin_fma(-ds[k], r[k], 1.0);
+#pragma unroll
+  for (int k = 0; k < N; k++) r[k] = __builtin_fma(r[k], e[k], r[k]);
+#pragma unroll
+  for (int k = 0; k < N; k++) e[k] = __builtin_fma(-ds[k], r[k], 1.0);
+#pragma unroll
+  for (int k = 0; k < N; k++) ns[k] = __builtin_amdgcn_div_scale(n[k], d[k], true, &f[k]);
+#pragma unroll
+  for (int k = 0; k < N; k++) r[k] = __builtin_fma(r[k], e[k], r[k]);
+#pragma unroll
+  for (int k = 0; k < N; k++) m[k] = ns[k] * r[k];
+#pragma unroll
+  for (int k = 0; k < N; k++) e[k] = __builtin_fma(-ds[k], m[k], ns[k]);
+#pragma unroll
+  for (int k = 0; k < N; k++) m[k] = __builtin_amdgcn_div_fmas(e[k], r[k], m[k], f[k]);
+#pragma unroll
+  for (int k = 0; k < N; k++) q[k] = __builtin_amdgcn_div_fixup(m[k], d[k], n[k]);
+#else
+#pragma unroll
+  for (int k = 0; k < N; k++) q[k] = n[k] / d[k];
+#endif
+}
+template <bool DIVB = false>
 RPT_DEV void div6(double n0, double n1, const RcpD& rx, double n2, double n3, const RcpD& ry, double n4, double n5,
                   const RcpD& rz, double& q0, double& q1, double& q2, double& q3, double& q4, double& q5) {
-  q0 = div_r(n0, rx); q1 = div_r(n1, rx);
-  q2 = div_r(n2, ry); q3 = div_r(n3, ry);
-  q4 = div_r(n4, rz); q5 = div_r(n5, rz);
+  if constexpr (DIVB) {
+    const double n[6] = {n0, n1, n2, n3, n4, n5}, d[6] = {rx.d, rx.d, ry.d, ry.d, rz.d, rz.d};
+    double q[6];
+    div_ieee<6>(n, d, q);
+    q0 = q[0]; q1 = q[1]; q2 = q[2]; q3 = q[3]; q4 = q[4]; q5 = q[5];
+  } else {
+    q0 = div_r(n0, rx); q1 = div_r(n1, rx);
+    q2 = div_r(n2, ry); q3 = div_r(n3, ry);
+    q4 = div_r(n4, rz); q5 = div_r(n5, rz);
+  }
 }
 RPT_DEV D3 operator/(D3 a, double s) {
   RcpD rc = rcp_make(s);
   return {div_r(a.x, rc), div_r(a.y, rc), div_r(a.z, rc)};
+}
+RPT_DEV D3 div3(D3 a, double s) {
+  const double n[3] = {a.x, a.y, a.z}, d[3] = {s, s, s};
+  double q[3];
+  div_ieee<3>(n, d, q);
+  return {q[0], q[1], q[2]};
 }
 RPT_DEV D3 cmul(D3 a, D3 b) { return {a.x * b.x, a.y * b.y, a.z * b.z}; }
 RPT_DEV double dot(D3 a, D3 b) { return (a.x * b.x + a.y * b.y) + a.z * b.z; }
 RPT_DEV double length2(D3 a) { return dot(a, a); }
 RPT_DEV double length(D3 a) { return sqrt(dot(a, a)); }
 RPT_DEV D3 normalize(D3 a) { return a / length(a); }
+RPT_DEV D3 normalize_b(D3 a) { return div3(a, length(a)); }
+template <bool DIVB> RPT_DEV D3 normalize_t(D3 a) {
+  if constexpr (DIVB) return normalize_b(a);
+  else return normalize(a);
+}
 RPT_DEV D3 cross(D3 a, D3 b) {
   return {a.y * b.z - a.z * b.y, a.z * b.x - a.x * b.z, a.x * b.y - a.y * b.x};
 }
```

New measurement: 1664 (median of 6 runs). 1.01x the previous value.
